# Shizheng-Wen/GAOT-3D

Hardware: AMD Instinct MI355X
Metric: mesh-points/sec fwd+bwd, 500K-pt DrivAerNet++ sample (higher is better)
Workload: dtype bf16; 1 GPU; configs[1]: one 500000-point car-like surface sample, latent 64x64x32, knn k=8 encoder + flipped decoder, C=32 P=2 d=256 h=8 F=1024 L=10 rope, attention dropout 0.1 (training mode), MSE + AdamW step; CSR build and geoembed stats inside the step (a decoder list that is the encoder's with its rows swapped shares the encoder's two lists); points=500000, edges=4000000, edges_decoder=4000000, layers=10, precision=bf16, points_per_gpu=500000, point_order=random

## Files before the change

gaot_3d_amd/_lib.py:

```python
from __future__ import annotations

import ctypes as C
import os

_HERE = os.path.dirname(os.path.abspath(__file__))
LIB_PATH = os.environ.get("GAOT_LIB") or os.path.join(_HERE, "lib", "libgaot3d_hip.so")

MAX_MLP_LAYERS = 5


class GaotError(RuntimeError):
    pass


class MlpT(C.Structure):
    _fields_ = [("n_hidden", C.c_int), ("hidden", C.c_int), ("channels", C.c_int),
                ("weight", C.c_void_p * MAX_MLP_LAYERS), ("bias", C.c_void_p * MAX_MLP_LAYERS)]


class MlpGradT(C.Structure):
    _fields_ = [("weight", C.c_void_p * MAX_MLP_LAYERS), ("bias", C.c_void_p * MAX_MLP_LAYERS)]


_lib = None

_p, _i, _i64, _sz, _f, _d = C.c_void_p, C.c_int, C.c_int64, C.c_size_t, C.c_float, C.c_double

SIGNATURES = {
    "gaot_abi_version": (_i, []),
    "gaot_last_error": (C.c_char_p, []),
    "gaot_launch_count": (_i64, [_i]),
    "gaot_csr_workspace_bytes": (_sz, [_i64, _i64]),
    "gaot_csr_build": (_i, [_p, _i, _i64, _i, _i64, _p, _p, _p, _p, _p, _sz, _p]),
    "gaot_gno_fwd_workspace_bytes": (_sz, [_i64, _i]),
    "gaot_gno_fwd": (_i, [C.POINTER(MlpT), _p, _p, _p, _p, _p, _p, _i64, _i64, _p, _i, _p, _sz, _p]),
    "gaot_gno_bwd_workspace_bytes": (_sz, [C.POINTER(MlpT), _i64, _i64]),
    "gaot_gno_bwd": (_i, [C.POINTER(MlpT), _p, _p, _p, _p, _p, _p, _p, _p, _i64, _i64, _i64, _p,
                          C.POINTER(MlpGradT), _i, _p, _sz, _p]),
    "gaot_gno_bwd_coords": (_i, [C.POINTER(MlpT), _p, _p, _p, _p, _p, _p, _p, _p, _i64, _i64, _i64, _p,
                                 C.POINTER(MlpGradT), _p, _i, _p, _sz, _p]),
    "gaot_geoembed_stats_workspace_bytes": (_sz, []),
    "gaot_geoembed_moments": (_i, [_p, _p, _p, _p, _i64, _p, _p]),
    "gaot_geoembed_from_moments": (_i, [_p, _i64, _p, _p, _sz, _p]),
    "gaot_geoembed_raw": (_i, [_p, _p, _p, _p, _i64, _p, _p, _p, _sz, _p]),
    "gaot_geoembed_finalize": (_i, [_p, _i64, _p, _i64, _p, _sz, _p]),
    "gaot_geoembed_from_moments_bwd_workspace_bytes": (_sz, [_i64]),
    "gaot_geoembed_from_moments_bwd": (_i, [_p, _p, _i64, _p, _p, _sz, _p]),
    "gaot_geoembed_moments_bwd": (_i, [_p, _p, _p, _p, _i64, _p, _p, _p, _p]),
    "gaot_gemm_workspace_bytes": (_sz, [_i64, _i64, _i64]),
    "gaot_gemm": (_i, [_p, _p, _p, _i64, _i64, _i64, _i64, _i64, _i64, _i, _i, _p, _i, _p, _i64, _p, _i, _p, _sz, _p]),
    "gaot_gemm_ex": (_i, [_p, _p, _p, _i64, _i64, _i64, _i64, _i64, _i64, _i, _i, _i, _i, _i, _p, _i, _p, _i64, _p, _i, _p,
                          _sz, _p]),
    "gaot_attn_fwd": (_i, [_p, _p, _p, _p, _p, _i64, _i64, _i64, _i64, _i, _i, _i, _i, _i, _f, _f, _p, _i, _i, _i, _p]),
    "gaot_attn_bwd": (_i, [_p] * 10 + [_i64] * 8 + [_i, _i, _i, _i, _i, _f, _f, _p, _i, _i, _i, _i, _p]),
    "gaot_attn_bwd_fused_f32_scratch_bytes": (_i64, [_i, _i, _i]),
    "gaot_attn_bwd_fused_f32": (_i, [_p] * 10 + [_i64] * 8 + [_i, _i, _i, _i, _i, _f, _f, _p, _i, _i, _i, _p, C.c_size_t, _p]),
    "gaot_attn_dropout_mask": (_i, [_p, _f, _i, _i, _i, _p, _p]),
    "gaot_dropout_seed_next": (_i, [_p, C.c_uint64, _p, _p]),
    "gaot_dropout_seed_block": (_i, [_p, C.c_uint64, _i, _p, _p]),
    "gaot_attn_bf16_image_bytes": (_sz, [_i, _i, _i, _i]),
    "gaot_rope_table": (_i, [_p, _i, _i, _p, _p]),
    "gaot_qkv_image": (_i, [_p, _p, _p, _i64, _i64, _i64, _i, _i, _i, _p, _f, _p]),
    "gaot_qkv_image_packed": (_i, [_p, _p, _p, _i64, _i64, _i64, _i64, _i, _i, _p, _f, _i, _p]),
    "gaot_pack_heads": (_i, [_p, _p, _i64, _i, _i, _i, _p, _p, _i, _i, _i, _p]),
    "gaot_attn_bwd_bf16_scratch_bytes": (_sz, [_i, _i, _i, _i]),
    "gaot_attn_bwd_bf16_fused_eligible": (_i, [_i, _i, _i, _i]),
    "gaot_attn_fwd_bf16": (_i, [_p, _p, _p, _p, _p, _i, _i, _i, _i, _i, _f, _f, _p, _i, _i, _p]),
    "gaot_attn_bwd_bf16": (_i, [_p, _p, _p, _p, _p, _p, _p, _p, _i, _i, _i, _i, _i, _f, _f, _p, _i, _i, _i, _p]),
    "gaot_rmsnorm_fwd": (_i, [_p, _p, _p, _p, _p, _i64, _i, _f, _p]),
    "gaot_rmsnorm_bwd_workspace_bytes": (_sz, [_i64, _i]),
    "gaot_rmsnorm_bwd": (_i, [_p, _p, _p, _p, _p, _p, _p, _i64, _i, _p, _sz, _p]),
    "gaot_rmsnorm_bwd2": (_i, [_p, _p, _p, _p, _p, _p, _p, _p, _i64, _i, _p, _sz, _p]),
    "gaot_colsum_workspace_bytes": (_sz, [_i64, _i64]),
    "gaot_colsum": (_i, [_p, _i64, _i64, _i64, _p, _p, _sz, _p]),
    "gaot_gemm_ex_partials": (_i, [_p, _p, _p, _i64, _i64, _i64, _i64, _i64, _i64, _i, _i, _i, _i, _i, _p, _sz, _p, _p, _p]),
    "gaot_rmsnorm_bwd_parts": (_i64, [_i64]),
    "gaot_colsum_parts": (_i64, [_i64]),
    "gaot_reduce_multi": (_i, [_p, _i, _p]),
    "gaot_rope": (_i, [_p, _i64, _i64, _i, _i, _i, _i, _p, _i, _p]),
    "gaot_swiglu_fwd": (_i, [_p, _p, _i64, _i, _p]),
    "gaot_swiglu_bwd": (_i, [_p, _p, _p, _i64, _i, _p]),
    "gaot_adamw_step": (_i, [_p, _i, _p, _p, _d, _d, _d, _d, _p]),
    "gaot_mlp2_fwd": (_i, [_p, _i64, _i, _i, _i, _p, _p, _p, _p, _p, _p]),
    "gaot_mlp2_bwd_workspace_bytes": (_sz, [_i, _i]),
    "gaot_mlp2_bwd": (_i, [_p, _i64, _i, _i, _i, _p, _p, _p, _p, _p, _p, _p, _p, _p, _sz, _p]),
    "gaot_knn_grid": (_i, [_p, _i64, _p, _p, _i, _p, _p]),
    "gaot_radius_grid_count": (_i, [_p, _i64, _p, _p, _f, _i, _p, _p]),
    "gaot_radius_grid_fill": (_i, [_p, _i64, _p, _p, _f, _i, _p, _p, _p, _p]),
    "gaot_knn_brute": (_i, [_p, _i64, _p, _i64, _i, _p, _p]),
    "gaot_radius_brute_count": (_i, [_p, _i64, _p, _i64, _f, _i, _p, _p]),
    "gaot_radius_brute_fill": (_i, [_p, _i64, _p, _i64, _f, _i, _p, _p, _p, _p]),
    "gaot_exclusive_scan_workspace_bytes": (_sz, [_i64]),
    "gaot_exclusive_scan_i32": (_i, [_p, _i64, _p, _p, _sz, _p]),
    "gaot_segment_cap_flags": (_i, [_p, _p, _i64, _i, _p, _p]),
    "gaot_unique_pair_flags": (_i, [_p, _p, _i64, _p, _p]),
    "gaot_random_keep_flags": (_i, [_p, _i64, _d, _p, _p]),
    "gaot_dropout": (_i, [_p, _p, _d, _i64, _p, _p]),
    "gaot_segment_random_cap_flags": (_i, [_p, _p, _p, _i64, _i, _p, _p]),
    "gaot_compact_pairs": (_i, [_p, _p, _p, _p, _i64, _p, _p, _p]),
    "gaot_cast_bf16": (_i, [_p, _p, _i64, _p]),
    "gaot_cast_bf16_multi": (_i, [_p, _i, _p]),
    "gaot_cast_bf16_transpose_multi": (_i, [_p, _p, _p, _i, _p]),
    "gaot_swiglu_fwd_bf16": (_i, [_p, _p, _i64, _i, _p]),
    "gaot_ffn_w13_swiglu": (_i, [_p, _p, _p, _p, _i64, _i64, _i64, _i, _p]),
    "gaot_ffn_w2_bwd_swiglu": (_i, [_p, _p, _p, _p, _i64, _i64, _i64, _i, _p]),
    "gaot_swiglu_bwd_bf16": (_i, [_p, _p, _p, _i64, _i, _p]),
    "gaot_ffn_packed_bytes": (_i64, [_i, _i]),
    "gaot_ffn_pack": (_i, [_p, _p, _i, _p, _i, _p]),
    "gaot_ffn_pack_multi": (_i, [_p, _i, _i, _i, _p]),
    "gaot_ffn_fwd": (_i, [_p, _p, _p, _i64, _p, _p, _p, _i64, _i, _p]),
    "gaot_norm_ffn_fwd": (_i, [_p, _i64, _p, _f, _p, _p, _p, _p, _i64, _i, _p]),
    "gaot_block_packed_bytes": (_i64, [_i]),
    "gaot_block_pack_multi": (_i, [_p, _i, _i, _p]),
    "gaot_block_tail_fwd": (_i, [_p, _i64, _p, _i64, _p, _f, _p, _p, _p, _p, _p, _i64, _i, _p]),
    "gaot_qkv_packed_bytes": (_i64, [_i64, _i]),
    "gaot_qkv_pack_multi": (_i, [_p, _i, _i64, _i, _p]),
    "gaot_norm_qkv_image": (_i, [_p, _i64, _p, _f, _p, _p, _p, _p, _i64, _i, _i, _i, _p, _f, _p]),
    "gaot_skip_packed_bytes": (_i64, []),
    "gaot_skip_pack_multi": (_i, [_p, _i, _p]),
    "gaot_cat_norm_qkv_image": (_i, [_p, _i64, _p, _i64, _p, _p, _p, _p, _f, _p, _p, _p, _p, _i64, _i, _i, _i, _p, _f, _p]),
    "gaot_norm_bwd_parts": (_i64, [_i64]),
    "gaot_ffn_bwd_norm": (_i, [_p, _p, _p, _p, _i64, _p, _p, _p, _p, _p, _p, _p, _i64, _i, _p]),
    "gaot_qkv_bwd_norm": (_i, [_p, _i64, _p, _p, _i64, _p, _p, _p, _p, _p, _p, _i64, _p]),
    "gaot_qkv_bwd_norm_cat": (_i, [_p, _i64, _p, _p, _i64, _p, _p, _p, _p, _p, _p, _p, _i, _p, _i64, _p]),
    "gaot_oproj_bwd_image": (_i, [_p, _p, _p, _i, _p, _p, _i64, _i, _p]),
    "gaot_ffn_bwd_dag": (_i, [_p, _p, _p, _p, _p, _p, _i64, _i, _p]),
    "gaot_ffn_bwd": (_i, [_p, _p, _p, _p, _p, _p, _p, _i, _i64, _i, _p]),
    "gaot_act_bwd": (_i, [_p, _p, _p, _i64, _i, _p]),
    "gaot_act_fwd": (_i, [_p, _p, _i64, _i, _p]),
    "gaot_axpy": (_i, [_p, _p, _f, _p, _i64, _i64, _p]),
    "gaot_stream_copy": (_i, [_p, _p, _i64, _p]),
    "gaot_stream_copy_ex": (_i, [_p, _p, _i64, _i, _p]),
    "gaot_patchify": (_i, [_p, _p, _i, _i, _i, _i, _i, _i, _i, _p]),
    "gaot_mse_workspace_bytes": (_sz, []),
    "gaot_mse_fwd": (_i, [_p, _p, _i64, _p, _p, _sz, _p]),
    "gaot_mse_bwd": (_i, [_p, _p, _i64, _p, _p, _p]),
    "gaot_gather_rows": (_i, [_p, _i64, _p, _i64, _i, _p, _i64, _p]),
    "gaot_segment_reduce": (_i, [_p, _i64, _p, _p, _i64, _i, _i, _p, _p, _p]),
    "gaot_segment_reduce_bwd": (_i, [_p, _p, _p, _p, _i64, _i64, _i, _i, _p, _p]),
    "gaot_segment_softmax_fwd": (_i, [_p, _p, _i64, _p, _p]),
    "gaot_segment_softmax_bwd": (_i, [_p, _p, _p, _i64, _p, _p]),
    "gaot_edge_coords": (_i, [_p, _p, _p, _p, _i64, _i, _p, _i64, _p]),
    "gaot_mul": (_i, [_p, _p, _i64, _i, _i, _p, _p]),
    "gaot_mul_rowsum": (_i, [_p, _p, _i64, _i, _p, _p]),
    "gaot_affine_cols": (_i, [_p, _p, _p, _i64, _i, _p, _p]),
    "gaot_scale_mix_fwd": (_i, [_p, _i, _p, _p, _p, _i64, _i, _p]),
    "gaot_scale_mix_bwd": (_i, [_p, _i, _p, _p, _p, _p, _i64, _i, _p]),
}


def load():
    global _lib
    if _lib is not None:
        return _lib
    if not os.path.exists(LIB_PATH):
        raise GaotError(f"{LIB_PATH} not found: build it with `python -c 'import __graft_entry__ as g; g.build()'` "
                        f"or `make -C gaot_3d_amd/csrc` (there is no CPU/PyTorch fallback)")
    lib = C.CDLL(LIB_PATH)
    for name, (res, args) in SIGNATURES.items():
        fn = getattr(lib, name)
        fn.restype = res
        fn.argtypes = args
    if lib.gaot_abi_version() != 11:
        raise GaotError("libgaot3d_hip.so ABI version mismatch")
    _lib = lib
    return lib


def check(rc: int, what: str):
    if rc != 0:
        msg = load().gaot_last_error()
        raise GaotError(f"{what} failed (code {rc}): {msg.decode() if msg else ''}")
```

gaot_3d_amd/functional.py:

```python
from __future__ import annotations

import os
from typing import List, Optional

import torch
from torch.autograd import Function

from . import ops
from ._lib import GaotError

Tensor = torch.Tensor


def _w2d(w: Tensor) -> Tensor:
    if w.dim() == 3:
        w = w[:, :, 0]
    return w if w.is_contiguous() else w.contiguous()


_WB_CACHE: dict = {}


def _wb_eligible(w: Tensor, prec: int) -> bool:
    n, k = w.shape
# ... 763 lines not shown
            packed = ops.qkv_pack_multi([wcat32], True)[0]
        spk = _SKIP_PACK_CACHE.get((wsk.data_ptr(), tuple(wsk.shape)))
        if spk is None:
            spk = ops.skip_pack_multi([wsk])[0]
        freqs, b, s, h, hkv, scale = image_spec
        img, xo, yb, rstd = ops.cat_norm_qkv_image(xa, xb, spk, bskip, norm_w, eps, packed, b, s, h, hkv, freqs, scale)
        out = torch.empty(1, dtype=torch.float32, device=x.device).expand(m, ntot)
        out._gaot_qkv_image = img
        ctx.save_for_backward(xa, xb, xo, norm_w, rstd, yb, _wb(wcat32, 1), packed, _wb(wsk, 1), spk)
        ctx.wparams, ctx.nparam, ctx.sparams = tuple(weights), norm_w, (wskip, bskip)
        ctx.meta = (x.shape, skip.shape, [w.shape for w in weights], ntot, wskip.shape)
        ctx.set_materialize_grads(False)
        return out, xo.view(x.shape)

    @staticmethod
    def backward(ctx, dqkv: Tensor, dres: Optional[Tensor] = None):
        xa, xb, xo, norm_w, rstd, yb, wcat, packed, wskb, spk = ctx.saved_tensors
        xshape, sshape, wshapes, ntot, wsshape = ctx.meta
        m = xa.shape[0]
        d = dqkv if dqkv.is_contiguous() else dqkv.contiguous()
        dwcat = _dw_gemm(d, yb, ntot, 256, m, ntot, 256, 1, ctx.wparams)
        dres2 = None if dres is None else dres.reshape(m, 256)
        dxa = dxb = None
        fused_dx = _NORM_BWD_FUSED and _CAT_BWD_DX and ctx.needs_input_grad[0] and (ctx.same or ctx.needs_input_grad[1])
        if fused_dx:
            dxo, dxa, dxb, dnw = ops.qkv_bwd_norm_cat(d, packed, xo, norm_w, rstd, dres2, spk, ctx.same, defer=ops.defer_ok((ctx.nparam,)))
        elif _NORM_BWD_FUSED:
            dxo, dnw = ops.qkv_bwd_norm(d, packed, xo, norm_w, rstd, dres2, None, defer=ops.defer_ok((ctx.nparam,)))
        else:
            dn = ops.gemm(d, wcat, m, 256, ntot, ntot, 256, False, False, precision=1)
            dxo, dnw = ops.rmsnorm_bwd(xo, norm_w, dn, rstd, dres2, defer=ops.defer_ok((ctx.nparam,)))
        n, k = 256, 512
        wsk, bsk = ctx.sparams
        if not fused_dx:
            dxa = ops.gemm(dxo, wskb, m, 256, n, n, k, False, False, precision=1) if (ctx.needs_input_grad[0] or ctx.same) else None
            if ctx.same and ctx.needs_input_grad[0]:
                dxa = ops.gemm(dxo, wskb[:, 256:], m, 256, n, n, k, False, False, residual=dxa, ldr=256, precision=1)
            else:
                dxb = ops.gemm(dxo, wskb[:, 256:], m, 256, n, n, k, False, False, precision=1) if ctx.needs_input_grad[1] else None
        dws = torch.empty(n, k, dtype=torch.float32, device=d.device)
        ops.gemm(dxo, xa, n, 256, m, n, 256, True, False, out=dws, ldc=k, precision=1)
        ops.gemm(dxo, xb, n, 256, m, n, 256, True, False, out=dws[:, 256:], ldc=k, precision=1)
        dbs = ops.colsum(dxo, m, n, n) if (bsk is not None and ctx.needs_input_grad[3]) else None
        dwl, col = [], 0
        for shp in wshapes:
            dwl.append(dwcat[col:col + shp[0]].view(shp))
            col += shp[0]
        return (None if dxa is None else dxa.view(xshape), None if dxb is None else dxb.view(sshape), dws.view(wsshape), dbs, dnw, None, None, *dwl)


class BlockTailFn(Function):

    @staticmethod
    def enabled() -> bool:
        return _FFN_FUSED and _NORM_FFN and _BLOCK_TAIL and ops.get_precision() == "bf16"

    @staticmethod
    def eligible(x: Tensor, wo: Tensor, norm_w: Tensor, w1: Tensor, w3: Tensor, w2: Tensor) -> bool:
        wo2 = _w2d(wo)
        return (BlockTailFn.enabled() and tuple(wo2.shape) == (256, 256) and wo2.dtype == torch.float32 and wo.requires_grad
                and NormFFNFn.eligible(x, norm_w, w1, w3, w2))

    @staticmethod
    def forward(ctx, o: Tensor, x: Tensor, wo: Tensor, norm_w: Tensor, eps: float, w1: Tensor, w3: Tensor, w2: Tensor, attn_dims=None):
        ctx.attn_dims = attn_dims if (attn_dims is not None and _OPROJ_BWD_IMAGE and attn_dims[2] == 8 and attn_dims[0] * attn_dims[1] == o.shape[0]) else None
        f, d = w1.shape
        o2 = o if o.is_contiguous() else o.contiguous()
        x2 = x if x.is_contiguous() else x.contiguous()
        wo2 = _w2d(wo)
        wcat32 = w1.new_empty(0).set_(w1.untyped_storage(), w1.storage_offset(), (2 * f, d), (d, 1))
        key = (wcat32.data_ptr(), tuple(wcat32.shape))
        packed, _has_bwd = _FFN_PACK_CACHE.get(key, (None, False))
        if packed is None or _WO_PACKED.get(key) != wo2.data_ptr():
            packed = ops.block_pack_multi([(wcat32, _w2d(w2), wo2)], f)[0]
        y, h, yb, rstd = ops.block_tail_fwd(o2, x2, norm_w, eps, packed, f)
        ctx.save_for_backward(o2, _wb(wo2, 1), h, norm_w, rstd, yb, packed)
        ctx.wparams = (w1, w3, w2)
        ctx.nparam, ctx.oparam = norm_w, wo
        ctx.meta = (f, d, w1.shape, w2.shape, wo.shape)
        return y

    @staticmethod
    def backward(ctx, dy: Tensor):
        o2, wob, h, norm_w, rstd, yb, packed = ctx.saved_tensors
        f, d, w1shape, w2shape, woshape = ctx.meta
        m = h.shape[0]
        dy2 = dy if dy.is_contiguous() else dy.contiguous()
        if _NORM_BWD_FUSED:
            dh, dag, u, dyb, dnw = ops.ffn_bwd_norm(yb, dy2, packed, f, h, norm_w, rstd, defer=ops.defer_ok((ctx.nparam,)))
        else:
            dn, dag, u, dyb = ops.ffn_bwd(yb, dy2, packed, f, True)
            dh, dnw = ops.rmsnorm_bwd(h, norm_w, dn, rstd, defer=ops.defer_ok((ctx.nparam,)))
        dw2 = _dw_gemm(dyb, u, d, f, m, d, f, 1, ctx.wparams[2:]).view(w2shape)
        dwcat = _dw_gemm(dag, yb, 2 * f, d, m, 2 * f, d, 1, ctx.wparams[:2])
        d_o = None
        if ctx.needs_input_grad[0]:
            if ctx.attn_dims is not None:
                b_, s_, h_, hkv_ = ctx.attn_dims
                img, delta = ops.oproj_bwd_image(dh, o2, packed, f, b_, s_, h_, hkv_)
                d_o = torch.empty(1, dtype=torch.float32, device=dh.device).expand(m, d)
                d_o._gaot_do_image = (img, delta)
            else:
                d_o = ops.gemm(dh, wob, m, d, d, d, d, False, False, precision=1)
        dwo = _dw_gemm(dh, o2, d, d, m, d, d, 1, (ctx.oparam,)).view(woshape)
        return d_o, (dh if ctx.needs_input_grad[1] else None), dwo, dnw, None, dwcat[:f].view(w1shape), dwcat[f:].view(w1shape), dw2, None


class Mlp2Fn(Function):

    @staticmethod
    def eligible(x: Tensor, fcs, non_linearity: str) -> bool:
        if len(fcs) != 2 or non_linearity != "gelu" or ops.get_precision() != "bf16" or not x.is_cuda:
            return False
        w1, w2 = _w2d(fcs[0].weight), _w2d(fcs[1].weight)
        return (x.shape[-1] == 32 and w1.shape[1] == 32 and w1.shape[0] in (64, 128, 256) and 1 <= w2.shape[0] <= 4
                and w2.shape[1] == w1.shape[0] and fcs[0].bias is not None and x.dtype == torch.float32)

    @staticmethod
    def forward(ctx, x: Tensor, w1: Tensor, b1: Tensor, w2: Tensor, b2: Optional[Tensor]):
        x2 = x.reshape(-1, x.shape[-1])
        if not x2.is_contiguous():
            x2 = x2.contiguous()
        w1c, w2c = _w2d(w1), _w2d(w2)
        out = ops.mlp2_forward(x2, w1c, b1, w2c, b2)
        ctx.save_for_backward(x2, w1c, b1, w2c)
        ctx.meta = (x.shape, w1.shape, w2.shape, b2 is not None)
        return out.view(*x.shape[:-1], w2c.shape[0])

    @staticmethod
    def backward(ctx, dout: Tensor):
        x2, w1c, b1, w2c = ctx.saved_tensors
        xshape, w1shape, w2shape, has_b2 = ctx.meta
        d = dout.reshape(x2.shape[0], w2c.shape[0])
        if not d.is_contiguous():
            d = d.contiguous()
        dx, dw1, db1, dw2 = ops.mlp2_backward(x2, w1c, b1, w2c, d)
        db2 = ops.colsum(d, d.shape[0], d.shape[1], d.shape[1]) if has_b2 else None
        return dx.view(xshape), dw1.view(w1shape), db1, dw2.view(w2shape), db2


class AddFn(Function):

    @staticmethod
    def forward(ctx, a: Tensor, b: Tensor, period: Optional[int]):
        ac = a if a.is_contiguous() else a.contiguous()
        bc = b if b.is_contiguous() else b.contiguous()
        ctx.period = period
        return ops.axpy(ac, bc, 1.0, period)

    @staticmethod
    def backward(ctx, g: Tensor):
        if ctx.period is not None and ctx.needs_input_grad[1]:
            raise GaotError("AddFn: gradient of a broadcast addend is not needed on the hot path")
        return g, (g if ctx.period is None else None), None


def add(a: Tensor, b: Tensor) -> Tensor:
    return AddFn.apply(a, b, None)


class PatchifyFn(Function):
    @staticmethod
    def forward(ctx, x: Tensor, b, d, h, w, p, c, to_tokens: bool):
        ctx.args = (b, d, h, w, p, c, to_tokens)
        xc = x if x.is_contiguous() else x.contiguous()
        return ops.patchify(xc, b, d, h, w, p, c, to_tokens)

    @staticmethod
    def backward(ctx, g: Tensor):
        b, d, h, w, p, c, to_tokens = ctx.args
        gc = g if g.is_contiguous() else g.contiguous()
        return ops.patchify(gc, b, d, h, w, p, c, not to_tokens), None, None, None, None, None, None, None


class MSELossFn(Function):
    @staticmethod
    def forward(ctx, pred: Tensor, target: Tensor):
        p = pred if pred.is_contiguous() else pred.contiguous()
        t = target if target.is_contiguous() else target.contiguous()
        if p.shape != t.shape:
            raise GaotError(f"mse_loss: shape mismatch {tuple(p.shape)} vs {tuple(t.shape)}")
        ctx.save_for_backward(p, t)
        return ops.mse_fwd(p, t)

    @staticmethod
    def backward(ctx, g: Tensor):
        p, t = ctx.saved_tensors
        gl = g if g.is_contiguous() else g.contiguous()
        return ops.mse_bwd(p, t, gl), None


def mse_loss(pred: Tensor, target: Tensor) -> Tensor:
    return MSELossFn.apply(pred, target)


def _adjacent(ws) -> bool:
    k = ws[0].shape[1]
    for a, b in zip(ws[:-1], ws[1:]):
        if b.shape[1] != k or not (a.is_contiguous() and b.is_contiguous()) or a.device != b.device:
            return False
        if b.data_ptr() != a.data_ptr() + a.numel() * a.element_size():
            return False
        if a.untyped_storage().data_ptr() != b.untyped_storage().data_ptr():
            return False
    return True


def colocate(params) -> None:
    ps = list(params)
    if _adjacent([_w2d(p.data) for p in ps]):
        return
    if torch.cuda.is_available() and torch.cuda.is_current_stream_capturing():
        raise GaotError("colocate: parameters must be co-located before the step is captured into a graph")
    with torch.no_grad():
        flat = torch.empty(sum(p.numel() for p in ps), dtype=ps[0].dtype, device=ps[0].device)
        off = 0
        for p in ps:
            v = flat[off:off + p.numel()].view(p.shape)
            v.copy_(p.data)
            p.data = v
            off += p.numel()


class MultiLinearFn(Function):

    @staticmethod
    def forward(ctx, x: Tensor, precision: Optional[int], image_spec, *weights: Tensor):
        ws = [_w2d(w) for w in weights]
        k = ws[0].shape[1]
        x2 = x.reshape(-1, k)
        if not x2.is_contiguous():
            x2 = x2.contiguous()
        m = x2.shape[0]
        ntot = sum(w.shape[0] for w in ws)
        ctx.fused = len(ws) > 1 and _adjacent(ws) and all(ctx.needs_input_grad[3 + i] for i in range(len(ws)))
        ctx.wparams = tuple(weights)
        if ctx.fused:
            wcat = _wb(ws[0].new_empty(0).set_(ws[0].untyped_storage(), ws[0].storage_offset(), (ntot, k), (k, 1)), precision)
            xb = bf16_copy_of(x, (m, k)) if wcat.dtype == torch.bfloat16 else None
            xa = xb if xb is not None else x2
            if image_spec is not None and xb is not None and k == 256 and ntot % 64 == 0:
                freqs, b, s, h, hkv, scale = image_spec
                img = ops.qkv_image(xb, wcat, m, b, s, h, hkv, freqs, scale)
                out = torch.empty(1, dtype=torch.float32, device=x.device).expand(m, ntot)
                out._gaot_qkv_image = img
                ctx.save_for_backward(xa, wcat)
                ctx.precision, ctx.xshape, ctx.wshapes = precision, x.shape, [w.shape for w in weights]
                return out
            out = torch.empty(m, ntot, dtype=torch.float32, device=x.device)
            ops.gemm(xa, wcat, m, ntot, k, k, k, False, True, out=out, ldc=ntot, precision=precision)
            ctx.save_for_backward(xa, wcat)
        else:
            out = torch.empty(m, ntot, dtype=torch.float32, device=x.device)
            col = 0
            for w in ws:
                n = w.shape[0]
                ops.gemm(x2, w, m, n, k, k, k, False, True, out=out[:, col:], ldc=ntot, precision=precision)
                col += n
            ctx.save_for_backward(x2, *ws)
        ctx.precision, ctx.xshape, ctx.wshapes = precision, x.shape, [w.shape for w in weights]
        return out

    @staticmethod
    def backward(ctx, dout: Tensor):
        x2, *ws = ctx.saved_tensors
        m, k = x2.shape
        d = dout if dout.is_contiguous() else dout.contiguous()
        ntot = d.shape[1]
        dx = None
        dws = []
        col = 0
        if ctx.fused:
            (wcat,) = ws
            if ctx.needs_input_grad[0]:
                dx = ops.gemm(d, wcat, m, k, ntot, ntot, k, False, False, precision=ctx.precision)
            dwcat = _dw_gemm(d, x2, ntot, k, m, ntot, k, ctx.precision, ctx.wparams)
            for shp in ctx.wshapes:
                n = shp[0]
                dws.append(dwcat[col:col + n].view(shp))
                col += n
            return (dx.view(ctx.xshape) if dx is not None else None, None, None, *dws)
        for i, w in enumerate(ws):
            n = w.shape[0]
            blk = d[:, col:]
            if ctx.needs_input_grad[0]:
                dx = ops.gemm(blk, w, m, k, n, ntot, k, False, False, residual=dx, ldr=k, precision=ctx.precision)
            dws.append(_dw_gemm(blk, x2, n, k, m, ntot, k, ctx.precision, ctx.wparams[i:i + 1]).view(ctx.wshapes[i])
                       if ctx.needs_input_grad[3 + i] else None)
            col += n
        return (dx.view(ctx.xshape) if dx is not None else None, None, None, *dws)


def multi_linear(x: Tensor, weights, precision: Optional[int] = None, image_spec=None) -> Tensor:
    return MultiLinearFn.apply(x, precision, image_spec, *weights)


def _same_view(a: Tensor, b: Tensor) -> bool:
    if a is b:
        return True
    ba, bb = (a._base if a._base is not None else a), (b._base if b._base is not None else b)
    return ba is bb and a.data_ptr() == b.data_ptr() and a.shape == b.shape and a.stride() == b.stride()


class CatLinearFn(Function):

    @staticmethod
    def forward(ctx, weight: Tensor, bias: Optional[Tensor], precision: Optional[int], *xs: Tensor):
        w = _w2d(weight)
        n, k = w.shape
        xs2 = [x if x.is_contiguous() else x.contiguous() for x in xs]
        if sum(x.shape[1] for x in xs2) != k:
            raise GaotError(f"cat_linear: inputs have {sum(x.shape[1] for x in xs2)} features, weight expects {k}")
        m = xs2[0].shape[0]
        if all(x.shape[1] > 64 and x.shape[1] % 8 == 0 for x in xs2):
            w = _wb(w, precision)
        y = None
        col = 0
        for i, x in enumerate(xs2):
            ki = x.shape[1]
            y = ops.gemm(x, w[:, col:], m, n, ki, ki, k, False, True, bias if i == 0 else None, 0, residual=y, ldr=n,
                         precision=precision)
            col += ki
        ctx.save_for_backward(w, *xs2)
        ctx.meta = (precision, weight.shape, bias is not None)
        ctx.dups = any(_same_view(xs[i], xs[j]) for i in range(len(xs)) for j in range(i))
        return y

    @staticmethod
    def backward(ctx, dy: Tensor):
        w, *xs = ctx.saved_tensors
        precision, wshape, has_bias = ctx.meta
        n, k = w.shape
        d = dy if dy.is_contiguous() else dy.contiguous()
        m = d.shape[0]
        dw = torch.empty(n, k, dtype=torch.float32, device=d.device) if ctx.needs_input_grad[0] else None
        dxs = []
        col = 0
        first = {}
        for i, x in enumerate(xs):
            ki = x.shape[1]
            key = (x.data_ptr(), tuple(x.shape))
            j = first.get(key)
            if ctx.needs_input_grad[3 + i] and j is not None and dxs[j] is not None and ctx.dups:
                dxs[j] = ops.gemm(d, w[:, col:], m, ki, n, n, k, False, False, residual=dxs[j], ldr=ki, precision=precision)
                dxs.append(None)
            else:
                dxs.append(ops.gemm(d, w[:, col:], m, ki, n, n, k, False, False, precision=precision)
                           if ctx.needs_input_grad[3 + i] else None)
                first.setdefault(key, i)
            if dw is not None:
                ops.gemm(d, x, n, ki, m, n, ki, True, False, out=dw[:, col:], ldc=k, precision=precision)
            col += ki
        db = ops.colsum(d, m, n, n) if (has_bias and ctx.needs_input_grad[1]) else None
        return (dw.view(wshape) if dw is not None else None, db, None, *dxs)


def cat_linear(xs, weight, bias=None, precision: Optional[int] = None) -> Tensor:
    return CatLinearFn.apply(weight, bias, precision, *xs)


class ScaleMixFn(Function):

    @staticmethod
    def forward(ctx, logits: Tensor, *xs: Tensor):
        xc = [x if x.is_contiguous() else x.contiguous() for x in xs]
        lg = logits if logits.is_contiguous() else logits.contiguous()
        out, w = ops.scale_mix_fwd(xc, lg)
        ctx.save_for_backward(w, *xc)
        return out

    @staticmethod
    def backward(ctx, dout: Tensor):
        w, *xs = ctx.saved_tensors
        d = dout if dout.is_contiguous() else dout.contiguous()
        dxs, dlog = ops.scale_mix_bwd(xs, w, d)
        return (dlog, *dxs)
```

gaot_3d_amd/model/layers/geoembed.py:

```python
from typing import Optional

import torch
import torch.nn as nn

from ... import edgeops as EO
from ... import functional as GF
from ... import ops
from .integral_transform import coords_need_grad, graph_for


class GeoStatFn(torch.autograd.Function):

    @staticmethod
    def forward(ctx, source_pos, query_pos, g):
        mom = ops.geoembed_moments(source_pos, query_pos, g)
        ctx.g = g
        ctx.save_for_backward(source_pos, query_pos, mom)
        return ops.geoembed_from_moments(mom)

    @staticmethod
    def backward(ctx, d):
        source_pos, query_pos, mom = ctx.saved_tensors
        g = ctx.g
        adj = ops.geoembed_from_moments_bwd(mom, d)
        ge, gq = ops.geoembed_moments_bwd(source_pos, query_pos, g, adj)
        gs = None
        if ctx.needs_input_grad[0]:
            gs, _ = EO.coord_grads_by_endpoint(ge, g, 0, None, source_pos.shape[0], query_pos.shape[0])
        return gs, (gq if ctx.needs_input_grad[1] else None), None


class GeometricEmbedding(nn.Module):
    def __init__(self, input_dim, output_dim, method="statistical", pooling="max", **kwargs):
        super().__init__()
        self.input_dim = input_dim
        self.output_dim = output_dim
        self.method = method.lower()
        self.pooling = pooling.lower()
        self.kwargs = kwargs
        if self.pooling not in ["max", "mean"]:
            raise ValueError(f"Unsupported pooling method: {self.pooling}. Supported methods: 'max', 'mean'.")
        if self.method == "statistical":
            self.mlp = nn.Sequential(nn.Linear(3 + 2 * input_dim, 64), nn.ReLU(), nn.Linear(64, output_dim))
        elif self.method == "pointnet":
            self.pointnet_mlp = nn.Sequential(nn.Linear(input_dim, 32), nn.ReLU(), nn.Linear(32, 32), nn.ReLU())
            self.fc = nn.Sequential(nn.Linear(32, output_dim))
        else:
            raise ValueError(f"Unknown method: {self.method}")

    def forward(self, source_pos, query_pos, edge_index, batch_source: Optional[torch.Tensor] = None,
                batch_query: Optional[torch.Tensor] = None, neighbors_counts: Optional[torch.Tensor] = None,
                graph=None, shard_group=None, sharded_queries_total: Optional[int] = None):
        if graph is None:
            graph = graph_for(edge_index.to(query_pos.device), source_pos.shape[0], query_pos.shape[0])
        coord_grad = coords_need_grad(source_pos, query_pos)
        if shard_group is not None and coord_grad:
            raise NotImplementedError("GeometricEmbedding: gradients with respect to the coordinates are not supported for "
                                      "point-sharded samples (shard_group); detach the coordinates")
        if self.method == "pointnet":
            if shard_group is not None and sharded_queries_total is None:
                return self._forward_pointnet_sharded(source_pos, query_pos, graph, shard_group)
            return self._forward_pointnet(source_pos, query_pos, graph)
        if shard_group is not None and sharded_queries_total is not None:
            feats = ops.geoembed_stats_sharded_queries(source_pos, query_pos, graph, shard_group, sharded_queries_total)
        elif shard_group is not None:
            import torch.distributed as dist
            mom = ops.geoembed_moments(source_pos, query_pos, graph)
            from ... import comm
            comm.run(lambda: dist.all_reduce(mom, op=dist.ReduceOp.SUM, group=shard_group), (mom,), "all_reduce")
            feats = ops.geoembed_from_moments(mom)
        elif coord_grad:
            feats = GeoStatFn.apply(source_pos, query_pos, graph)
        else:
            ent = graph.__dict__.get("_geo_feats")
            if (ent is not None and ent[0] is source_pos and ent[1] == source_pos._version and ent[2] is query_pos
                    and ent[3] == query_pos._version):
                feats = ent[4]
            else:
                feats = ops.geoembed_from_moments(ops.geoembed_moments(source_pos, query_pos, graph))
                graph.__dict__["_geo_feats"] = (source_pos, source_pos._version, query_pos, query_pos._version, feats)
        h = GF.linear(feats, self.mlp[0].weight, self.mlp[0].bias, act="relu", precision=0)
        return GF.linear(h, self.mlp[2].weight, self.mlp[2].bias, precision=0)

    def _forward_pointnet_sharded(self, source_pos, query_pos, g, group):
        from ...sharding import GlobalSegmentMaxFn, GlobalSegmentMeanFn
        nq = query_pos.shape[0]
        rp = g.by_dst.rowptr
        deg = (rp[1:] - rp[:-1]).to(torch.float32)
        if g.by_dst.num_edges == 0:
            local = torch.zeros(nq, 32, dtype=query_pos.dtype, device=query_pos.device)
        else:
            c = EO.edge_coords(source_pos, query_pos, g, 1)
            h = GF.linear(c, self.pointnet_mlp[0].weight, self.pointnet_mlp[0].bias, act="relu", precision=0)
            h = GF.linear(h, self.pointnet_mlp[2].weight, self.pointnet_mlp[2].bias, act="relu", precision=0)
            local = EO.SegmentReduceFn.apply(h, g, EO.MAX if self.pooling == "max" else EO.MEAN)
        if self.pooling == "max":
            pooled, gdeg = GlobalSegmentMaxFn.apply(local, deg, group)
        else:
            pooled = GlobalSegmentMeanFn.apply(local, deg, group)
            gdeg = deg.clone()
            import torch.distributed as dist
            from ... import comm
            comm.run(lambda: dist.all_reduce(gdeg, op=dist.ReduceOp.SUM, group=group), (gdeg,), "all_reduce")
        po = GF.linear(pooled, self.fc[0].weight, self.fc[0].bias, precision=0)
        return EO.RowScaleFn.apply(po, (gdeg > 0).to(torch.float32))

    def _forward_pointnet(self, source_pos, query_pos, g):
        nq = query_pos.shape[0]
        if g.by_dst.num_edges == 0:
            return torch.zeros(nq, self.output_dim, dtype=query_pos.dtype, device=query_pos.device)
        c = EO.EdgeOffsetFn.apply(source_pos, query_pos, g)
        h = GF.linear(c, self.pointnet_mlp[0].weight, self.pointnet_mlp[0].bias, act="relu", precision=0)
        h = GF.linear(h, self.pointnet_mlp[2].weight, self.pointnet_mlp[2].bias, act="relu", precision=0)
        pooled = EO.SegmentReduceFn.apply(h, g, EO.MAX if self.pooling == "max" else EO.MEAN)
        po = GF.linear(pooled, self.fc[0].weight, self.fc[0].bias, precision=0)
        rp = g.by_dst.rowptr
        has = (rp[1:] > rp[:-1]).to(torch.float32)
        return EO.RowScaleFn.apply(po, has)
```

gaot_3d_amd/model/layers/magno.py:

```python
from dataclasses import dataclass, field
from typing import Any, List, Optional, Tuple, Union

import torch
import torch.nn as nn

from ... import functional as GF
from ...data import coalesce_edges, knn_edges_bruteforce, radius_edges_bruteforce
from .geoembed import GeometricEmbedding
from ...graph import apply_neighbor_sampling
from .integral_transform import IntegralTransform, graph_for
from .mlp import ChannelMLP, LinearChannelMLP


@dataclass
class MAGNOConfig:
    use_gno: bool = True
    gno_coord_dim: int = 2
    gno_radius: float = 0.033
    lifting_channels: int = 16
    encoder_feature_attr: Any = "x"
    in_gno_channel_mlp_hidden_layers: list = field(default_factory=lambda: [64, 64, 64])
    in_gno_transform_type: str = "linear"
    projection_channels: int = 256
    out_gno_channel_mlp_hidden_layers: list = field(default_factory=lambda: [64, 64])
    out_gno_transform_type: str = "linear"
    mlp_type: str = "channel"
    scales: list = field(default_factory=lambda: [1.0])
    use_scale_weights: bool = False
    use_graph_cache: bool = True
    gno_use_torch_cluster: bool = False
    gno_use_torch_scatter: str = True
    node_embedding: bool = False
    use_attn: Optional[bool] = None
    attention_type: str = "cosine"
    use_geoembed: Any = field(default_factory=lambda: [True, True])
    embedding_method: str = "statistical"
    pooling: str = "max"
    sampling_strategy: Optional[str] = None
    max_neighbors: Optional[int] = None
    sample_ratio: Optional[float] = None
    neighbor_strategy: Any = "radius"
    k_neighbors: int = 1
    precompute_edges: bool = True
    asynchronous_graph_building: bool = False


def parse_neighbor_strategy(neighbor_strategy: Union[str, List[str]]) -> Tuple[str, str]:
    if isinstance(neighbor_strategy, str):
        return neighbor_strategy, neighbor_strategy
    if isinstance(neighbor_strategy, (list, tuple)) and len(neighbor_strategy) == 2:
        return neighbor_strategy[0], neighbor_strategy[1]
    raise ValueError(f"neighbor_strategy must be str or list of length 2, got {neighbor_strategy}")


def parse_geoembed_strategy(use_geoembed: Union[bool, List[bool]]) -> Tuple[bool, bool]:
    if isinstance(use_geoembed, bool):
        return use_geoembed, use_geoembed
    if isinstance(use_geoembed, (list, tuple)) and len(use_geoembed) == 2:
        return use_geoembed[0], use_geoembed[1]
    raise ValueError(f"use_geoembed must be bool or list of length 2, got {use_geoembed}")


def _per_graph(fn, phys_pos, batch_idx_phys, latent_pos, batch_idx_latent):
    nb = int(batch_idx_phys.max().item()) + 1 if batch_idx_phys.numel() else 1
    out = []
    for b in range(nb):
        pm = (batch_idx_phys == b).nonzero(as_tuple=True)[0]
        lm = (batch_idx_latent == b).nonzero(as_tuple=True)[0]
        e = fn(phys_pos[pm], latent_pos[lm])
        out.append((e, pm, lm))
    return out


def get_neighbor_strategy(neighbor_strategy: str, phys_pos, batch_idx_phys, latent_tokens_pos, batch_idx_latent,
                          radius: float, k_neighbors: int = 1, is_decoder: bool = False, latent_dims=None):
    if phys_pos.is_cuda:
        from ... import graph as device_graph
        return device_graph.get_neighbor_strategy(neighbor_strategy, phys_pos, batch_idx_phys, latent_tokens_pos,
                                                  batch_idx_latent, radius, k_neighbors, is_decoder, latent_dims=latent_dims)

    def enc(strategy, p, l):
        knn = rad = None
        if strategy in ("knn", "bidirectional"):
            knn = knn_edges_bruteforce(p, l, k_neighbors)
        if strategy in ("radius", "bidirectional"):
            rad = radius_edges_bruteforce(p, l, radius, 32, centers="latent")
        if strategy == "knn":
            return knn
        if strategy == "radius":
            return rad
        if strategy == "bidirectional":
            return coalesce_edges(torch.cat([knn, rad], dim=1), l.shape[0])
        raise ValueError(f"Unknown encoder strategy: {strategy}")

    def dec(strategy, p, l):
        if strategy == "reverse":
            return enc("bidirectional", p, l).flip(0)
        knn = rad = None
        if strategy in ("knn", "bidirectional"):
            knn = knn_edges_bruteforce(p, l, k_neighbors).flip(0)
        if strategy in ("radius", "bidirectional"):
            rad = radius_edges_bruteforce(p, l, radius, 32, centers="phys")
        if strategy == "knn":
            return knn
        if strategy == "radius":
            return rad
        if strategy == "bidirectional":
            return coalesce_edges(torch.cat([knn, rad], dim=1), p.shape[0])
        raise ValueError(f"Unknown decoder strategy: {strategy}")

    parts = _per_graph((lambda p, l: dec(neighbor_strategy, p, l)) if is_decoder else
                       (lambda p, l: enc(neighbor_strategy, p, l)),
                       phys_pos, batch_idx_phys, latent_tokens_pos, batch_idx_latent)
    outs = []
    for e, pm, lm in parts:
        if is_decoder:
            outs.append(torch.stack([lm[e[0]], pm[e[1]]]))
        else:
            outs.append(torch.stack([pm[e[0]], lm[e[1]]]))
    return torch.cat(outs, dim=1) if outs else torch.empty((2, 0), dtype=torch.long, device=phys_pos.device)


def _make_mlp(mlp_type, layers):
    if mlp_type == "linear":
        return LinearChannelMLP(layers=layers)
    if len(layers) == 2:
        return ChannelMLP(in_channels=layers[0], out_channels=layers[1], n_layers=1)
    return ChannelMLP(in_channels=layers[0], out_channels=layers[-1], hidden_channels=layers[1], n_layers=len(layers) - 1,
                      n_dim=1)


def _check_unsupported(cfg: MAGNOConfig):
    if cfg.sampling_strategy not in (None, "max_neighbors", "ratio"):
        raise ValueError(f"Invalid sampling strategy: {cfg.sampling_strategy}")


def _sample(module, edge_index, num_query):
    if module.sampling_strategy is None:
        return edge_index
    from ...graph import apply_neighbor_sampling
    return apply_neighbor_sampling(edge_index, num_query, edge_index.device, module.sampling_strategy, module.max_neighbors,
                                   module.sample_ratio, module.training)


def _sum_scales(outs):
    acc = outs[0]
    for o in outs[1:]:
        acc = GF.add(acc, o)
    return acc


def _make_scale_weighting(coord_dim, num_scales):
    return nn.Sequential(nn.Linear(coord_dim, 16), nn.ReLU(), nn.Linear(16, num_scales))


def _mix_scales(module, outs, pos):
    if len(outs) == 1:
        return outs[0]
    if not module.use_scale_weights:
        return _sum_scales(outs)
    sw = module.scale_weighting
    h = GF.linear(pos, sw[0].weight, sw[0].bias, act="relu", precision=0)
    logits = GF.linear(h, sw[2].weight, sw[2].bias, precision=0)
    return GF.ScaleMixFn.apply(logits, *outs)


class MAGNOEncoder(nn.Module):
    def __init__(self, in_channels, out_channels, gno_config: MAGNOConfig):
        super().__init__()
        _check_unsupported(gno_config)
        self.sampling_strategy = gno_config.sampling_strategy
        self.max_neighbors = gno_config.max_neighbors
        self.sample_ratio = gno_config.sample_ratio
        self.gno_radius = gno_config.gno_radius
        self.scales = gno_config.scales
        self.lifting_channels = gno_config.lifting_channels
        self.coord_dim = gno_config.gno_coord_dim
        self.feature_attr_name = gno_config.encoder_feature_attr
        self.precompute_edges = gno_config.precompute_edges
        self.mlp_type = gno_config.mlp_type
        self.encoder_strategy, self.decoder_strategy = parse_neighbor_strategy(gno_config.neighbor_strategy)
        self.k_neighbors = gno_config.k_neighbors
        self.use_gno = gno_config.use_gno
        if self.use_gno:
            kin = self.coord_dim * 2
            if gno_config.in_gno_transform_type in ("nonlinear", "nonlinear_kernelonly"):
                kin += in_channels
            layers = [kin] + list(gno_config.in_gno_channel_mlp_hidden_layers) + [self.lifting_channels]
            self.gno = IntegralTransform(channel_mlp_layers=layers, transform_type=gno_config.in_gno_transform_type,
                                         use_attn=gno_config.use_attn, coord_dim=self.coord_dim,
                                         attention_type=gno_config.attention_type)
            self.lifting = _make_mlp(gno_config.mlp_type, [in_channels, self.lifting_channels])
        else:
            self.gno = None
            self.lifting = None
        self.use_geoembed = parse_geoembed_strategy(gno_config.use_geoembed)[0]
        if self.use_geoembed:
            self.geoembed = GeometricEmbedding(input_dim=self.coord_dim, output_dim=self.lifting_channels,
                                               method=gno_config.embedding_method, pooling=gno_config.pooling)
            self.recovery = _make_mlp(gno_config.mlp_type, [2 * self.lifting_channels, self.lifting_channels])
        self.use_scale_weights = gno_config.use_scale_weights
        if self.use_scale_weights:
            self.num_scales = len(self.scales)
            self.scale_weighting = _make_scale_weighting(self.coord_dim, self.num_scales)
            self.scale_weight_activation = nn.Softmax(dim=-1)

    def _features(self, batch):
        names = self.feature_attr_name if isinstance(self.feature_attr_name, (list, tuple)) else [self.feature_attr_name]
        feats = []
        for a in names:
            f = getattr(batch, a, None)
            if f is None:
                if self.use_gno:
                    raise AttributeError(f"MAGNOEncoder requires feature attribute '{a}' but it was not found in the batch.")
            else:
                feats.append(f)
        return feats

    def forward(self, batch, latent_tokens_pos: torch.Tensor, latent_tokens_batch_idx: torch.Tensor) -> torch.Tensor:
        phys_pos = batch.pos
        device = phys_pos.device
        num_graphs = batch.num_graphs
        m_per_graph = latent_tokens_pos.shape[0] // num_graphs
        phys_feat = self._features(batch)
        lifted = None
        if self.use_gno:
            if len(self.lifting.fcs) == 1 and not (self.training and getattr(self.lifting, "dropout_p", 0.0) > 0.0):
                lifted = GF.cat_linear(phys_feat, self.lifting.fcs[0].weight, self.lifting.fcs[0].bias, precision=0)
            else:
                lifted = self.lifting.forward_rows(phys_feat[0] if len(phys_feat) == 1 else torch.cat(phys_feat, dim=1))
        outs = []
        for si, scale in enumerate(self.scales):
            if self.precompute_edges:
                attr = f"encoder_edge_index_s{si}"
                if not hasattr(batch, attr):
                    raise AttributeError(f"Batch object missing pre-computed '{attr}'")
                edge_index = getattr(batch, attr).to(device)
            else:
                edge_index = get_neighbor_strategy(self.encoder_strategy, phys_pos, batch.batch, latent_tokens_pos,
                                                   latent_tokens_batch_idx, self.gno_radius * scale, self.k_neighbors,
                                                   False, latent_dims=getattr(self, "latent_dims", None)).to(device)
            edge_index = _sample(self, edge_index, latent_tokens_pos.shape[0])
            g = graph_for(edge_index, phys_pos.shape[0], latent_tokens_pos.shape[0],
                          batch if self.sampling_strategy is None else None, ("enc", si))
            enc = self.gno(y_pos=phys_pos, x_pos=latent_tokens_pos, edge_index=edge_index, f_y=lifted,
                           graph=g) if self.use_gno else None
            shard_group = getattr(self, "_shard_group", None)
            if shard_group is not None and enc is not None:
                from ...sharding import GlobalSegmentMeanFn
                deg = (g.by_dst.rowptr[1:] - g.by_dst.rowptr[:-1]).to(enc.dtype)
                enc = GlobalSegmentMeanFn.apply(enc, deg, shard_group)
            geo = self.geoembed(phys_pos, latent_tokens_pos, edge_index, graph=g, shard_group=shard_group) \
                if self.use_geoembed else None
            if enc is not None and geo is not None:
                enc = GF.cat_linear([enc, geo], self.recovery.fcs[0].weight, self.recovery.fcs[0].bias, precision=0)
            elif enc is None and geo is not None:
                enc = geo
            elif enc is None:
                raise ValueError("GNO and GeoEmbed are both disabled. No encoding will be performed.")
            outs.append(enc)
        out = _mix_scales(self, outs, latent_tokens_pos)
        return out.view(num_graphs, m_per_graph, self.lifting_channels)


class MAGNODecoder(nn.Module):
    def __init__(self, in_channels, out_channels, gno_config: MAGNOConfig):
        super().__init__()
        _check_unsupported(gno_config)
        self.sampling_strategy = gno_config.sampling_strategy
        self.max_neighbors = gno_config.max_neighbors
        self.sample_ratio = gno_config.sample_ratio
        self.gno_radius = gno_config.gno_radius
        self.scales = gno_config.scales
        self.coord_dim = gno_config.gno_coord_dim
        self.in_channels = in_channels
        self.out_channels = out_channels
        self.use_geoembed = parse_geoembed_strategy(gno_config.use_geoembed)[1]
        self.use_scale_weights = gno_config.use_scale_weights
        self.precompute_edges = gno_config.precompute_edges
        self.mlp_type = gno_config.mlp_type
        self.encoder_strategy, self.decoder_strategy = parse_neighbor_strategy(gno_config.neighbor_strategy)
        self.k_neighbors = gno_config.k_neighbors
        kin = self.coord_dim * 2
        if gno_config.out_gno_transform_type in ("nonlinear", "nonlinear_kernelonly"):
            kin += in_channels
        layers = [kin] + list(gno_config.out_gno_channel_mlp_hidden_layers) + [in_channels]
        self.gno = IntegralTransform(channel_mlp_layers=layers, transform_type=gno_config.out_gno_transform_type,
                                     use_attn=gno_config.use_attn, coord_dim=self.coord_dim,
                                     attention_type=gno_config.attention_type)
        self.projection = _make_mlp(gno_config.mlp_type, [in_channels, gno_config.projection_channels, out_channels])
        if self.use_geoembed:
            self.geoembed = GeometricEmbedding(input_dim=self.coord_dim, output_dim=in_channels,
                                               method=gno_config.embedding_method, pooling=gno_config.pooling)
            self.recovery = _make_mlp(gno_config.mlp_type, [2 * in_channels, in_channels])
        if self.use_scale_weights:
            self.num_scales = len(self.scales)
            self.scale_weighting = _make_scale_weighting(self.coord_dim, self.num_scales)
            self.scale_weight_activation = nn.Softmax(dim=-1)

    def forward(self, rndata_flat, phys_pos_query, batch_idx_phys_query, latent_tokens_pos, latent_tokens_batch_idx,
                batch=None) -> torch.Tensor:
        device = rndata_flat.device
        outs = []
        for si, scale in enumerate(self.scales):
            if self.precompute_edges:
                attr = f"decoder_edge_index_s{si}"
                if not hasattr(batch, attr):
                    raise AttributeError(f"Batch object missing pre-computed '{attr}'")
                edge_index = getattr(batch, attr).to(device)
            else:
                edge_index = get_neighbor_strategy(self.decoder_strategy, phys_pos_query, batch_idx_phys_query,
                                                   latent_tokens_pos, latent_tokens_batch_idx, self.gno_radius * scale,
                                                   self.k_neighbors, True,
                                                   latent_dims=getattr(self, "latent_dims", None)).to(device)
            edge_index = _sample(self, edge_index, phys_pos_query.shape[0])
            g = graph_for(edge_index, latent_tokens_pos.shape[0], phys_pos_query.shape[0],
                          batch if self.sampling_strategy is None else None, ("dec", si))
            dec = self.gno(y_pos=latent_tokens_pos, x_pos=phys_pos_query, edge_index=edge_index, f_y=rndata_flat, graph=g)
            if self.use_geoembed:
                sg = getattr(self, "_shard_group", None)
                if sg is not None:
                    total = getattr(batch, "shard", (0, 0, 0, 0, phys_pos_query.shape[0]))[4]
                    geo = self.geoembed(latent_tokens_pos, phys_pos_query, edge_index, graph=g, shard_group=sg,
                                        sharded_queries_total=total)
                else:
                    geo = self.geoembed(latent_tokens_pos, phys_pos_query, edge_index, graph=g)
                dec = GF.cat_linear([dec, geo], self.recovery.fcs[0].weight, self.recovery.fcs[0].bias, precision=0)
            outs.append(dec)
        return self.projection.forward_rows(_mix_scales(self, outs, phys_pos_query))
```

gaot_3d_amd/ops.py:

```python
from __future__ import annotations

import ctypes as C
import functools
import os
from dataclasses import dataclass
from typing import List, Optional, Sequence, Tuple

import torch

from . import _lib
from ._lib import GaotError, MlpGradT, MlpT, check

Tensor = torch.Tensor


_raw_stream = getattr(torch._C, "_cuda_getCurrentRawStream", None)


def _stream() -> C.c_void_p:
    if _raw_stream is not None:
        return C.c_void_p(_raw_stream(torch.cuda.current_device()))
    return C.c_void_p(torch.cuda.current_stream().cuda_stream)


# ... 893 lines not shown
        raise GaotError("norm_qkv_image: fp32 [b * s, 256] input expected")
    nw = _req(norm_weight, torch.float32, "norm_weight")
    img = _ws(lib.gaot_attn_bf16_image_bytes(b, s, h, hkv), x.device)
    yb = torch.empty(rows, 256, dtype=torch.bfloat16, device=x.device)
    rstd = torch.empty(rows, dtype=torch.float32, device=x.device)
    table = rope_table(freqs, s) if freqs is not None else None
    with _timed("norm_qkv_image"):
        check(lib.gaot_norm_qkv_image(_ptr(x), x.stride(0), _ptr(nw), float(eps), _ptr(packed), _ptr(img), _ptr(yb), _ptr(rstd), rows, s, h, hkv,
                                      _ptr(table), _qscale(scale), _stream()), "gaot_norm_qkv_image")
    return img, yb, rstd


def _finish_parts(part: Tensor, n: int, parts: int, lanes: int, defer: bool) -> Tensor:
    out = torch.empty(n, dtype=torch.float32, device=part.device)
    if defer:
        _defer(part, out, n, parts, lanes)
        return out
    arr = (_ReduceDesc * 1)()
    arr[0].part, arr[0].out, arr[0].n, arr[0].parts, arr[0].lanes = part.data_ptr(), out.data_ptr(), n, parts, lanes
    check(_lib.load().gaot_reduce_multi(arr, 1, _stream()), "gaot_reduce_multi")
    return out


def ffn_bwd_norm(yb: Tensor, dy: Tensor, packed: Tensor, f: int, h: Tensor, norm_weight: Tensor, rstd: Tensor, defer: bool = False):
    lib = _lib.load()
    rows = yb.shape[0]
    if yb.dtype != torch.bfloat16 or not yb.is_contiguous() or yb.shape[1] != 256:
        raise GaotError("ffn_bwd_norm: contiguous bf16 [rows, 256] input expected")
    if dy.dtype != torch.float32 or not dy.is_contiguous() or tuple(dy.shape) != (rows, 256):
        raise GaotError("ffn_bwd_norm: contiguous fp32 [rows, 256] gradient expected")
    if h.dtype != torch.float32 or tuple(h.shape) != (rows, 256) or h.stride(1) != 1:
        raise GaotError("ffn_bwd_norm: fp32 [rows, 256] norm input expected")
    nw = _req(norm_weight, torch.float32, "norm_weight")
    dev = yb.device
    dag = torch.empty(rows, 2 * f, dtype=torch.bfloat16, device=dev)
    u = torch.empty(rows, f, dtype=torch.bfloat16, device=dev)
    dyb = torch.empty(rows, 256, dtype=torch.bfloat16, device=dev)
    dh = torch.empty(rows, 256, dtype=torch.float32, device=dev)
    parts = int(lib.gaot_norm_bwd_parts(rows))
    part = torch.empty(parts, 256, dtype=torch.float32, device=dev)
    with _timed("ffn_bwd_norm"):
        check(lib.gaot_ffn_bwd_norm(_ptr(yb), _ptr(dy), _ptr(packed), _ptr(h), h.stride(0), _ptr(nw), _ptr(rstd), _ptr(dag), _ptr(u), _ptr(dyb),
                                    _ptr(dh), _ptr(part), rows, int(f), _stream()), "gaot_ffn_bwd_norm")
    return dh, dag, u, dyb, _finish_parts(part, 256, parts, 32, defer)


def qkv_bwd_norm(dqkv: Tensor, packed: Tensor, x: Tensor, norm_weight: Tensor, rstd: Tensor, dres: Optional[Tensor] = None,
                 dtap: Optional[Tensor] = None, defer: bool = False):
    lib = _lib.load()
    rows, n = dqkv.shape
    if dqkv.dtype != torch.float32 or not dqkv.is_contiguous() or n % 256:
        raise GaotError("qkv_bwd_norm: contiguous fp32 [rows, N] gradient with N a multiple of 256 expected")
    if x.dtype != torch.float32 or tuple(x.shape) != (rows, 256) or x.stride(1) != 1:
        raise GaotError("qkv_bwd_norm: fp32 [rows, 256] norm input expected")
    nw = _req(norm_weight, torch.float32, "norm_weight")
    dres = None if dres is None else _req(dres, torch.float32, "dres")
    dtap = None if dtap is None else _req(dtap, torch.float32, "dtap")
    dev = dqkv.device
    dx = torch.empty(rows, 256, dtype=torch.float32, device=dev)
    parts = int(lib.gaot_norm_bwd_parts(rows))
    part = torch.empty(parts, 256, dtype=torch.float32, device=dev)
    with _timed("qkv_bwd_norm"):
        check(lib.gaot_qkv_bwd_norm(_ptr(dqkv), n, _ptr(packed), _ptr(x), x.stride(0), _ptr(nw), _ptr(rstd), _ptr(dres), _ptr(dtap), _ptr(dx),
                                    _ptr(part), rows, _stream()), "gaot_qkv_bwd_norm")
    return dx, _finish_parts(part, 256, parts, 32, defer)


def qkv_bwd_norm_cat(dqkv: Tensor, packed: Tensor, x: Tensor, norm_weight: Tensor, rstd: Tensor, dres: Optional[Tensor], skip_packed: Tensor,
                     same: bool, defer: bool = False):
    lib = _lib.load()
    rows, n = dqkv.shape
    if dqkv.dtype != torch.float32 or not dqkv.is_contiguous() or n % 256:
        raise GaotError("qkv_bwd_norm_cat: contiguous fp32 [rows, N] gradient with N a multiple of 256 expected")
    if x.dtype != torch.float32 or tuple(x.shape) != (rows, 256) or x.stride(1) != 1:
        raise GaotError("qkv_bwd_norm_cat: fp32 [rows, 256] norm input expected")
    if skip_packed.numel() != int(lib.gaot_skip_packed_bytes()):
        raise GaotError("qkv_bwd_norm_cat: skip_packed is not a skip_pack_multi image")
    nw = _req(norm_weight, torch.float32, "norm_weight")
    dres = None if dres is None else _req(dres, torch.float32, "dres")
    dev = dqkv.device
    dx = torch.empty(rows, 256, dtype=torch.float32, device=dev)
    dxa = torch.empty(rows, 256, dtype=torch.float32, device=dev)
    dxb = None if same else torch.empty(rows, 256, dtype=torch.float32, device=dev)
    parts = int(lib.gaot_norm_bwd_parts(rows))
    part = torch.empty(parts, 256, dtype=torch.float32, device=dev)
    with _timed("qkv_bwd_norm_cat"):
        check(lib.gaot_qkv_bwd_norm_cat(_ptr(dqkv), n, _ptr(packed), _ptr(x), x.stride(0), _ptr(nw), _ptr(rstd), _ptr(dres), _ptr(skip_packed),
                                        _ptr(dx), _ptr(dxa), _ptr(dxb), int(bool(same)), _ptr(part), rows, _stream()), "gaot_qkv_bwd_norm_cat")
    return dx, dxa, dxb, _finish_parts(part, 256, parts, 32, defer)


def oproj_bwd_image(dh: Tensor, attn_out: Tensor, packed: Tensor, f: int, b: int, s: int, h: int, hkv: int):
    lib = _lib.load()
    rows = dh.shape[0]
    if h != 8 or rows != b * s or any(t.dtype != torch.float32 or not t.is_contiguous() or tuple(t.shape) != (rows, 256) for t in (dh, attn_out)):
        raise GaotError("oproj_bwd_image: contiguous fp32 [b * s, 256] tensors and 8 heads of 32 expected")
    scratch = attn_bwd_scratch(b, s, h, hkv, dh.device)
    delta = torch.empty(b, h, s, dtype=torch.float32, device=dh.device)
    with _timed("oproj_bwd_image"):
        check(lib.gaot_oproj_bwd_image(_ptr(dh), _ptr(attn_out), _ptr(packed), int(f), _ptr(scratch), _ptr(delta), rows, int(s), _stream()),
              "gaot_oproj_bwd_image")
    return scratch, delta


def norm_ffn_fwd(h: Tensor, norm_weight: Tensor, eps: float, packed: Tensor, f: int):
    lib = _lib.load()
    if h.dtype != torch.float32 or h.dim() != 2 or h.shape[1] != 256 or h.stride(1) != 1:
        raise GaotError("norm_ffn_fwd: fp32 [rows, 256] input expected")
    nw = _req(norm_weight, torch.float32, "norm_weight")
    rows = h.shape[0]
    y = torch.empty(rows, 256, dtype=torch.float32, device=h.device)
    yb = torch.empty(rows, 256, dtype=torch.bfloat16, device=h.device)
    rstd = torch.empty(rows, dtype=torch.float32, device=h.device)
    with _timed("norm_ffn_fwd"):
        check(lib.gaot_norm_ffn_fwd(_ptr(h), h.stride(0), _ptr(nw), float(eps), _ptr(packed), _ptr(y), _ptr(yb), _ptr(rstd), rows, int(f),
                                    _stream()), "gaot_norm_ffn_fwd")
    return y, yb, rstd


def ffn_bwd_dag(xb: Tensor, dy: Tensor, packed: Tensor, f: int, want_dyb: bool = True):
    lib = _lib.load()
    if xb.dtype != torch.bfloat16 or not xb.is_contiguous() or xb.shape[1] != 256:
        raise GaotError("ffn_bwd_dag: contiguous bf16 [rows, 256] input expected")
    rows = xb.shape[0]
    if dy.dtype != torch.float32 or not dy.is_contiguous() or tuple(dy.shape) != (rows, 256):
        raise GaotError("ffn_bwd_dag: contiguous fp32 [rows, 256] gradient expected")
    dag = torch.empty(rows, 2 * f, dtype=torch.bfloat16, device=xb.device)
    u = torch.empty(rows, f, dtype=torch.bfloat16, device=xb.device)
    dyb = torch.empty(rows, 256, dtype=torch.bfloat16, device=xb.device) if want_dyb else None
    with _timed("ffn_bwd_dag"):
        check(lib.gaot_ffn_bwd_dag(_ptr(xb), _ptr(dy), _ptr(packed), _ptr(dag), _ptr(u), _ptr(dyb), rows, int(f), _stream()), "gaot_ffn_bwd_dag")
    return dag, u, dyb


def ffn_bwd(xb: Tensor, dy: Tensor, packed: Tensor, f: int, add_dy: bool, want_dyb: bool = True):
    lib = _lib.load()
    if xb.dtype != torch.bfloat16 or not xb.is_contiguous() or xb.shape[1] != 256:
        raise GaotError("ffn_bwd: contiguous bf16 [rows, 256] input expected")
    rows = xb.shape[0]
    if dy.dtype != torch.float32 or not dy.is_contiguous() or tuple(dy.shape) != (rows, 256):
        raise GaotError("ffn_bwd: contiguous fp32 [rows, 256] gradient expected")
    dag = torch.empty(rows, 2 * f, dtype=torch.bfloat16, device=xb.device)
    u = torch.empty(rows, f, dtype=torch.bfloat16, device=xb.device)
    dyb = torch.empty(rows, 256, dtype=torch.bfloat16, device=xb.device) if want_dyb else None
    dx = torch.empty(rows, 256, dtype=torch.float32, device=xb.device)
    with _timed("ffn_bwd"):
        check(lib.gaot_ffn_bwd(_ptr(xb), _ptr(dy), _ptr(packed), _ptr(dag), _ptr(u), _ptr(dyb), _ptr(dx), int(add_dy), rows, int(f), _stream()),
              "gaot_ffn_bwd")
    return dx, dag, u, dyb


def ffn_w2_bwd_swiglu(dyb: Tensor, w2t: Tensor, ag: Tensor, f: int) -> Tensor:
    lib = _lib.load()
    if any(t.dtype != torch.bfloat16 or not t.is_contiguous() for t in (dyb, w2t, ag)):
        raise GaotError("ffn_w2_bwd_swiglu: contiguous bf16 operands expected")
    dag = torch.empty_like(ag)
    with _timed("ffn_w2_bwd_swiglu"):
        check(lib.gaot_ffn_w2_bwd_swiglu(_ptr(dyb), _ptr(w2t), _ptr(ag), _ptr(dag), dyb.shape[0], dyb.shape[1], w2t.shape[1], int(f),
                                         _stream()), "gaot_ffn_w2_bwd_swiglu")
    return dag


def swiglu_bwd_bf16(ag: Tensor, du: Tensor, f: int) -> Tensor:
    lib = _lib.load()
    dag = torch.empty_like(ag)
    check(lib.gaot_swiglu_bwd_bf16(_ptr(ag), _ptr(du), _ptr(dag), ag.shape[0], f, _stream()), "gaot_swiglu_bwd_bf16")
    return dag


def patchify(src: Tensor, b: int, d: int, h: int, w: int, p: int, c: int, to_tokens: bool) -> Tensor:
    lib = _lib.load()
    dst = torch.empty_like(src)
    check(lib.gaot_patchify(_ptr(src), _ptr(dst), b, d, h, w, p, c, int(to_tokens), _stream()), "gaot_patchify")
    return dst


def mse_fwd(pred: Tensor, target: Tensor) -> Tensor:
    lib = _lib.load()
    loss = torch.empty((), dtype=torch.float32, device=pred.device)
    ws = _ws(lib.gaot_mse_workspace_bytes(), pred.device)
    check(lib.gaot_mse_fwd(_ptr(pred), _ptr(target), pred.numel(), _ptr(loss), _ptr(ws), ws.numel(), _stream()),
          "gaot_mse_fwd")
    return loss


def mse_bwd(pred: Tensor, target: Tensor, grad_loss: Tensor) -> Tensor:
    lib = _lib.load()
    dp = torch.empty_like(pred)
    check(lib.gaot_mse_bwd(_ptr(pred), _ptr(target), pred.numel(), _ptr(grad_loss), _ptr(dp), _stream()), "gaot_mse_bwd")
    return dp


def geoembed_stats_sharded_queries(source_pos: Tensor, query_pos: Tensor, g: BipartiteGraph, group, num_queries_total: int) -> Tensor:
    import torch.distributed as dist
    lib = _lib.load()
    source_pos = _req(source_pos, torch.float32, "source_pos")
    query_pos = _req(query_pos, torch.float32, "query_pos")
    if source_pos.shape[1] != 3:
        raise GaotError("geoembed statistical features: coord_dim must be 3 on the HIP path")
    q = g.num_dst
    feat = torch.empty(q, 9, dtype=torch.float32, device=query_pos.device)
    sums = torch.empty(18, dtype=torch.float64, device=query_pos.device)
    ws = _ws(lib.gaot_geoembed_stats_workspace_bytes(), query_pos.device)
    check(lib.gaot_geoembed_raw(_ptr(source_pos), _ptr(query_pos), _ptr(g.by_dst.rowptr), _ptr(g.by_dst.other), q, _ptr(feat),
                                _ptr(sums), _ptr(ws), ws.numel(), _stream()), "gaot_geoembed_raw")
    if group is not None:
        from . import comm
        comm.run(lambda: dist.all_reduce(sums, op=dist.ReduceOp.SUM, group=group), (sums,), "all_reduce")
    check(lib.gaot_geoembed_finalize(_ptr(feat), q, _ptr(sums), int(num_queries_total), _ptr(ws), ws.numel(), _stream()),
          "gaot_geoembed_finalize")
    return feat


def geoembed_moments(source_pos: Tensor, query_pos: Tensor, g: BipartiteGraph) -> Tensor:
    lib = _lib.load()
    source_pos = _req(source_pos, torch.float32, "source_pos")
    query_pos = _req(query_pos, torch.float32, "query_pos")
    if source_pos.shape[1] != 3:
        raise GaotError("geoembed statistical features: coord_dim must be 3 on the HIP path")
    mom = torch.empty(g.num_dst, 12, dtype=torch.float64, device=query_pos.device)
    check(lib.gaot_geoembed_moments(_ptr(source_pos), _ptr(query_pos), _ptr(g.by_dst.rowptr), _ptr(g.by_dst.other), g.num_dst,
                                    _ptr(mom), _stream()), "gaot_geoembed_moments")
    return mom


def geoembed_from_moments(mom: Tensor) -> Tensor:
    lib = _lib.load()
    q = mom.shape[0]
    feat = torch.empty(q, 9, dtype=torch.float32, device=mom.device)
    ws = _ws(lib.gaot_geoembed_stats_workspace_bytes(), mom.device)
    check(lib.gaot_geoembed_from_moments(_ptr(mom), q, _ptr(feat), _ptr(ws), ws.numel(), _stream()), "gaot_geoembed_from_moments")
    return feat


def geoembed_from_moments_bwd(mom: Tensor, grad_feat: Tensor) -> Tensor:
    lib = _lib.load()
    q = mom.shape[0]
    grad_feat = _req(grad_feat, torch.float32, "grad_features")
    adj = torch.empty(q, 12, dtype=torch.float64, device=mom.device)
    ws = _ws(lib.gaot_geoembed_from_moments_bwd_workspace_bytes(q), mom.device)
    check(lib.gaot_geoembed_from_moments_bwd(_ptr(mom), _ptr(grad_feat), q, _ptr(adj), _ptr(ws), ws.numel(), _stream()),
          "gaot_geoembed_from_moments_bwd")
    return adj


def geoembed_moments_bwd(source_pos: Tensor, query_pos: Tensor, g: BipartiteGraph, adj: Tensor):
    lib = _lib.load()
    source_pos = _req(source_pos, torch.float32, "source_pos")
    query_pos = _req(query_pos, torch.float32, "query_pos")
    ge = torch.empty(g.by_dst.num_edges, 3, dtype=torch.float32, device=query_pos.device)
    gq = torch.empty(g.num_dst, 3, dtype=torch.float32, device=query_pos.device)
    check(lib.gaot_geoembed_moments_bwd(_ptr(source_pos), _ptr(query_pos), _ptr(g.by_dst.rowptr), _ptr(g.by_dst.other),
                                        g.num_dst, _ptr(adj), _ptr(ge), _ptr(gq), _stream()), "gaot_geoembed_moments_bwd")
    return ge, gq


def _ptr_array(ts):
    arr = (C.c_void_p * len(ts))()
    for i, t in enumerate(ts):
        arr[i] = _ptr(t).value
    return arr


def scale_mix_fwd(xs, logits: Tensor):
    lib = _lib.load()
    n, c = xs[0].shape
    out = torch.empty_like(xs[0])
    w = torch.empty(n, len(xs), dtype=torch.float32, device=out.device)
    check(lib.gaot_scale_mix_fwd(_ptr_array(xs), len(xs), _ptr(logits), _ptr(out), _ptr(w), n, c, _stream()),
          "gaot_scale_mix_fwd")
    return out, w


def scale_mix_bwd(xs, w: Tensor, dout: Tensor):
    lib = _lib.load()
    n, c = xs[0].shape
    dxs = [torch.empty_like(x) for x in xs]
    dlog = torch.empty_like(w)
    check(lib.gaot_scale_mix_bwd(_ptr_array(xs), len(xs), _ptr(w), _ptr(dout), _ptr_array(dxs), _ptr(dlog), n, c,
                                 _stream()), "gaot_scale_mix_bwd")
    return dxs, dlog


def mlp2_forward(x: Tensor, w1: Tensor, b1: Tensor, w2: Tensor, b2: Optional[Tensor]) -> Tensor:
    lib = _lib.load()
    rows, hid, oc = x.shape[0], w1.shape[0], w2.shape[0]
    out = torch.empty(rows, oc, dtype=torch.float32, device=x.device)
    check(lib.gaot_mlp2_fwd(_ptr(x), rows, x.shape[1], hid, oc, _ptr(w1), _ptr(b1), _ptr(w2), _ptr(b2), _ptr(out), _stream()),
          "gaot_mlp2_fwd")
    return out


def mlp2_backward(x: Tensor, w1: Tensor, b1: Tensor, w2: Tensor, dout: Tensor):
    lib = _lib.load()
    rows, hid, oc = x.shape[0], w1.shape[0], w2.shape[0]
    dx = torch.empty_like(x)
    dw1, db1, dw2 = torch.empty_like(w1), torch.empty_like(b1), torch.empty_like(w2)
    ws = _ws(lib.gaot_mlp2_bwd_workspace_bytes(hid, oc), x.device)
    check(lib.gaot_mlp2_bwd(_ptr(x), rows, x.shape[1], hid, oc, _ptr(w1), _ptr(b1), _ptr(w2), _ptr(dout), _ptr(dx), _ptr(dw1),
                            _ptr(db1), _ptr(dw2), _ptr(ws), ws.numel(), _stream()), "gaot_mlp2_bwd")
    return dx, dw1, db1, dw2


def launch_count_reset() -> None:
    _lib.load().gaot_launch_count(1)


def launch_count() -> int:
    return int(_lib.load().gaot_launch_count(0))
```

include/gaot3d_hip.h:

```cpp
#ifndef GAOT3D_HIP_H
#define GAOT3D_HIP_H

#include <stddef.h>
#include <stdint.h>

#ifdef __cplusplus
extern "C" {
#endif

#define GAOT_OK 0
#define GAOT_ERR_ARG 1
#define GAOT_ERR_LAUNCH 2
#define GAOT_ERR_UNSUPPORTED 3

#define GAOT_ABI_VERSION 11
#define GAOT_MAX_MLP_LAYERS 5

typedef void* gaot_stream_t;

int gaot_abi_version(void);
const char* gaot_last_error(void);
int64_t gaot_launch_count(int reset);

size_t gaot_csr_workspace_bytes(int64_t num_edges, int64_t num_rows);
int gaot_csr_build(const void* edge_index, int index_is_i64, int64_t num_edges, int sort_row, int64_t num_rows,
                   int32_t* rowptr, int32_t* perm, int32_t* key_sorted, int32_t* other_sorted, void* workspace,
                   size_t workspace_bytes, gaot_stream_t stream);

typedef struct {
    int n_hidden;
    int hidden;
    int channels;
    const float* weight[GAOT_MAX_MLP_LAYERS];
    const float* bias[GAOT_MAX_MLP_LAYERS];
} gaot_mlp_t;

typedef struct {
    float* weight[GAOT_MAX_MLP_LAYERS];
    float* bias[GAOT_MAX_MLP_LAYERS];
} gaot_mlp_grad_t;

size_t gaot_gno_fwd_workspace_bytes(int64_t num_edges, int channels);
int gaot_gno_fwd(const gaot_mlp_t* mlp , const float* y_pos, const float* x_pos, const float* f_y,
                 const int32_t* src_sorted, const int32_t* dst_sorted, const int32_t* rowptr_dst, int64_t num_edges,
                 int64_t num_queries, float* out ,
                 int precision ,
                 void* workspace, size_t workspace_bytes, gaot_stream_t stream);

size_t gaot_gno_bwd_workspace_bytes(const gaot_mlp_t* mlp , int64_t num_edges, int64_t num_queries);
int gaot_gno_bwd(const gaot_mlp_t* mlp , const float* y_pos, const float* x_pos, const float* f_y,
                 const float* grad_out , const int32_t* rowptr_dst,
                 const int32_t* src_sorted , const int32_t* dst_sorted ,
                 const int32_t* rowptr_src, int64_t num_edges, int64_t num_sources, int64_t num_queries,
                 float* grad_f_y , const gaot_mlp_grad_t* grads ,
                 int precision, void* workspace, size_t workspace_bytes, gaot_stream_t stream);
int gaot_gno_bwd_coords(const gaot_mlp_t* mlp , const float* y_pos, const float* x_pos, const float* f_y,
                        const float* grad_out, const int32_t* rowptr_dst, const int32_t* src_sorted, const int32_t* dst_sorted,
                        const int32_t* rowptr_src, int64_t num_edges, int64_t num_sources, int64_t num_queries,
                        float* grad_f_y, const gaot_mlp_grad_t* grads , float* grad_edge_coords ,
                        int precision, void* workspace, size_t workspace_bytes, gaot_stream_t stream);

size_t gaot_geoembed_stats_workspace_bytes(void);
int gaot_geoembed_moments(const float* source_pos, const float* query_pos, const int32_t* rowptr_dst,
                          const int32_t* src_sorted, int64_t num_queries, double* moments, gaot_stream_t stream);
int gaot_geoembed_from_moments(const double* moments, int64_t num_queries, float* features, void* workspace,
                               size_t workspace_bytes, gaot_stream_t stream);
int gaot_geoembed_raw(const float* source_pos, const float* query_pos, const int32_t* rowptr_dst, const int32_t* src_sorted,
                      int64_t num_queries, float* features, double* colsums, void* workspace, size_t workspace_bytes,
                      gaot_stream_t stream);
int gaot_geoembed_finalize(float* features, int64_t num_queries, const double* colsums, int64_t num_queries_total,
                           void* workspace, size_t workspace_bytes, gaot_stream_t stream);
size_t gaot_geoembed_from_moments_bwd_workspace_bytes(int64_t num_queries);
int gaot_geoembed_from_moments_bwd(const double* moments, const float* grad_features, int64_t num_queries,
                                   double* grad_moments, void* workspace, size_t workspace_bytes, gaot_stream_t stream);
int gaot_geoembed_moments_bwd(const float* source_pos, const float* query_pos, const int32_t* rowptr_dst,
                              const int32_t* src_sorted, int64_t num_queries, const double* grad_moments,
                              float* grad_edge , float* grad_query , gaot_stream_t stream);

size_t gaot_gemm_workspace_bytes(int64_t M, int64_t N, int64_t K);
int gaot_gemm(const float* A, const float* B, float* C, int64_t M, int64_t N, int64_t K, int64_t lda, int64_t ldb,
              int64_t ldc, int a_trans, int b_trans, const float* bias, int act, const float* residual, int64_t ldr,
              float* preact, int precision, void* workspace, size_t workspace_bytes, gaot_stream_t stream);
int gaot_gemm_ex(const void* A, const void* B, void* C, int64_t M, int64_t N, int64_t K, int64_t lda, int64_t ldb,
                 int64_t ldc, int a_trans, int b_trans, int a_bf16, int b_bf16, int c_bf16, const float* bias, int act,
                 const float* residual, int64_t ldr, float* preact, int precision, void* workspace,
                 size_t workspace_bytes, gaot_stream_t stream);

int gaot_attn_fwd(const float* q, const float* k, const float* v, float* o, float* lse, int64_t ldq, int64_t ldk,
                  int64_t ldv, int64_t ldo, int B, int S, int H, int HKV, int head_dim, float scale, float dropout_p,
                  const unsigned long long* dropout_seed, int head0, int heads_total, int precision, gaot_stream_t stream);
int gaot_attn_bwd(const float* q, const float* k, const float* v, const float* o, const float* d_o, const float* lse,
                  float* delta, float* dq, float* dk, float* dv, int64_t ldq, int64_t ldk, int64_t ldv, int64_t ldo,
                  int64_t lddo, int64_t lddq, int64_t lddk, int64_t lddv, int B, int S, int H, int HKV, int head_dim,
                  float scale, float dropout_p, const unsigned long long* dropout_seed, int head0, int heads_total,
                  int precision, int phase_mask , gaot_stream_t stream);
int64_t gaot_attn_bwd_fused_f32_scratch_bytes(int B, int S, int H);
int gaot_attn_bwd_fused_f32(const float* q, const float* k, const float* v, const float* o, const float* d_o, const float* lse,
                            float* delta, float* dq, float* dk, float* dv, int64_t ldq, int64_t ldk, int64_t ldv, int64_t ldo,
                            int64_t lddo, int64_t lddq, int64_t lddk, int64_t lddv, int B, int S, int H, int HKV, int head_dim,
                            float scale, float dropout_p, const unsigned long long* dropout_seed, int head0, int heads_total,
                            int run_delta, void* scratch, size_t scratch_bytes, gaot_stream_t stream);
int gaot_attn_dropout_mask(const unsigned long long* dropout_seed, float dropout_p, int B, int H, int S,
                           unsigned char* keep, gaot_stream_t stream);
int gaot_dropout_seed_next(unsigned long long* state, unsigned long long stride, unsigned long long* out,
                           gaot_stream_t stream);
int gaot_dropout_seed_block(unsigned long long* state, unsigned long long stride, int n, unsigned long long* out, gaot_stream_t stream);

int gaot_rope_table(const float* freqs, int S, int half_dim, float* table, gaot_stream_t stream);
int gaot_qkv_image(const void* x_bf16, const void* w_bf16, void* image, int64_t rows, int64_t lda, int64_t ldw, int S, int H,
                   int HKV, const float* rope_table, float qscale, gaot_stream_t stream);
int gaot_qkv_image_packed(const void* x_bf16, const void* w_bf16, void* packed, int64_t rows, int64_t lda, int64_t ldw,
                          int64_t pos0, int H, int HKV, const float* rope_table, float qscale, int world, gaot_stream_t stream);
int gaot_pack_heads(void* rows_buf, void* blocks_buf, int64_t rows, int ld, int world, int nseg, const int* col0,
                    const int* width, int rows_dtype, int blocks_dtype, int to_blocks, gaot_stream_t stream);
size_t gaot_attn_bf16_image_bytes(int B, int S, int H, int HKV);
size_t gaot_attn_bwd_bf16_scratch_bytes(int B, int S, int H, int HKV);
int gaot_attn_bwd_bf16_fused_eligible(int B, int S, int H, int HKV);
int gaot_attn_fwd_bf16(const float* qkv, const float* rope_freqs, void* qkv_image, float* o, float* lse, int B, int S,
                       int H, int HKV, int head_dim, float scale, float dropout_p,
                       const unsigned long long* dropout_seed, int head0, int heads_total, gaot_stream_t stream);
int gaot_attn_bwd_bf16(const void* qkv_image, const float* o, const float* d_o, const float* lse, void* do_image,
                       float* delta, float* dqkv, const float* rope_freqs, int B, int S, int H, int HKV, int head_dim,
                       float scale, float dropout_p, const unsigned long long* dropout_seed, int head0, int heads_total,
                       int phase_mask, gaot_stream_t stream);

int gaot_rmsnorm_fwd(const float* x, const float* weight, float* y, float* rstd, void* y_bf16 , int64_t rows, int dim, float eps,
                     gaot_stream_t stream);
size_t gaot_rmsnorm_bwd_workspace_bytes(int64_t rows, int dim);
int gaot_rmsnorm_bwd(const float* x, const float* weight, const float* dy, const float* rstd, const float* dx_add,
                     float* dx, float* dweight, int64_t rows, int dim, void* workspace, size_t workspace_bytes,
                     gaot_stream_t stream);
int gaot_rmsnorm_bwd2(const float* x, const float* weight, const float* dy, const float* rstd, const float* dx_add,
                      const float* dx_add2, float* dx, float* dweight, int64_t rows, int dim, void* workspace, size_t workspace_bytes,
                      gaot_stream_t stream);
size_t gaot_colsum_workspace_bytes(int64_t M, int64_t N);
int gaot_colsum(const float* x, int64_t M, int64_t N, int64_t ld, float* out, void* workspace, size_t workspace_bytes,
                gaot_stream_t stream);
typedef struct {
    const float* part;
    float* out;
    int64_t n;
    int32_t parts;
    int32_t lanes;
} gaot_reduce_desc_t;
int gaot_gemm_ex_partials(const void* A, const void* B, void* C, int64_t M, int64_t N, int64_t K, int64_t lda, int64_t ldb,
                          int64_t ldc, int a_trans, int b_trans, int a_bf16, int b_bf16, int precision, void* workspace,
                          size_t workspace_bytes, int* splits_out, int* lanes_out, gaot_stream_t stream);
int64_t gaot_rmsnorm_bwd_parts(int64_t rows);
int64_t gaot_colsum_parts(int64_t M);
int gaot_reduce_multi(const gaot_reduce_desc_t* descs, int count, gaot_stream_t stream);
int gaot_rope(float* x, int64_t rows, int64_t ld, int col0, int nheads, int head_dim, int seq_len, const float* freqs,
              int inverse, gaot_stream_t stream);
int gaot_swiglu_fwd(const float* ag, float* u, int64_t rows, int F, gaot_stream_t stream);
int gaot_swiglu_bwd(const float* ag, const float* du, float* dag, int64_t rows, int F, gaot_stream_t stream);
int gaot_cast_bf16(const float* src, void* dst, int64_t n, gaot_stream_t stream);
typedef struct {
    const float* src;
    void* dst;
    int64_t numel;
} gaot_cast_tensor_t;
int gaot_cast_bf16_multi(const gaot_cast_tensor_t* tensors, int num_tensors, gaot_stream_t stream);
int gaot_cast_bf16_transpose_multi(const gaot_cast_tensor_t* tensors, const int* rows, const int* cols, int num_tensors,
                                   gaot_stream_t stream);
int gaot_swiglu_fwd_bf16(const void* ag, void* u, int64_t rows, int F, gaot_stream_t stream);
int gaot_ffn_w13_swiglu(const void* x_bf16, const void* w13_bf16, void* ag, void* u, int64_t rows, int64_t lda, int64_t ldw, int F,
                        gaot_stream_t stream);
int gaot_swiglu_bwd_bf16(const void* ag, const void* du, void* dag, int64_t rows, int F, gaot_stream_t stream);
int gaot_ffn_w2_bwd_swiglu(const void* dy_bf16, const void* w2t_bf16, const void* ag, void* dag, int64_t rows, int64_t lda,
                           int64_t ldw, int F, gaot_stream_t stream);
int64_t gaot_ffn_packed_bytes(int F, int with_backward);
int gaot_ffn_pack(const float* w13, const float* w2, int F, void* packed, int with_backward, gaot_stream_t stream);
typedef struct {
    const float* w13;
    const float* w2;
    void* packed;
} gaot_ffn_pack_t;
int gaot_ffn_pack_multi(const gaot_ffn_pack_t* items, int num, int F, int with_backward, gaot_stream_t stream);
int gaot_ffn_fwd(const void* x_bf16, const void* packed, const float* residual, int64_t ldr, float* y, void* ag, void* u, int64_t rows,
                 int F, gaot_stream_t stream);
int gaot_norm_ffn_fwd(const float* h, int64_t ldh, const float* norm_weight, float eps, const void* packed, float* y, void* yb,
                      float* rstd, int64_t rows, int F, gaot_stream_t stream);
typedef struct {
    const float* w13;
    const float* w2;
    const float* wo;
    void* packed;
} gaot_block_pack_t;
int64_t gaot_block_packed_bytes(int F);
int gaot_block_pack_multi(const gaot_block_pack_t* items, int num, int F, gaot_stream_t stream);
int gaot_block_tail_fwd(const float* attn_out, int64_t ldo, const float* x, int64_t ldx, const float* norm_weight, float eps,
                        const void* packed, float* h, float* y, void* yb, float* rstd, int64_t rows, int F, gaot_stream_t stream);
typedef struct {
    const float* w;
    void* packed;
} gaot_qkv_pack_t;
int64_t gaot_qkv_packed_bytes(int64_t N, int with_backward);
int gaot_qkv_pack_multi(const gaot_qkv_pack_t* items, int num, int64_t N, int with_backward, gaot_stream_t stream);
int gaot_norm_qkv_image(const float* x, int64_t ldx, const float* norm_weight, float eps, const void* packed, void* image, void* yb,
                        float* rstd, int64_t rows, int S, int H, int HKV, const float* rope_table, float qscale, gaot_stream_t stream);
int64_t gaot_skip_packed_bytes(void);
int gaot_skip_pack_multi(const gaot_qkv_pack_t* items, int num, gaot_stream_t stream);
int gaot_cat_norm_qkv_image(const float* xa, int64_t ldxa, const float* xb, int64_t ldxb, const void* skip_packed, const float* skip_bias,
                            float* x_out, const float* norm_weight, float eps, const void* packed, void* image, void* yb, float* rstd,
                            int64_t rows, int S, int H, int HKV, const float* rope_table, float qscale, gaot_stream_t stream);
int64_t gaot_norm_bwd_parts(int64_t rows);
int gaot_ffn_bwd_norm(const void* yb, const float* dy, const void* packed, const float* h, int64_t ldh, const float* norm_weight,
                      const float* rstd, void* dag, void* u, void* dyb, float* dh, float* dw_part, int64_t rows, int F, gaot_stream_t stream);
int gaot_qkv_bwd_norm(const float* dqkv, int64_t N, const void* packed, const float* x, int64_t ldx, const float* norm_weight,
                      const float* rstd, const float* dres, const float* dtap, float* dx, float* dw_part, int64_t rows, gaot_stream_t stream);
int gaot_qkv_bwd_norm_cat(const float* dqkv, int64_t N, const void* packed, const float* x, int64_t ldx, const float* norm_weight,
                          const float* rstd, const float* dres, const void* skip_packed, float* dx, float* dxa, float* dxb, int same,
                          float* dw_part, int64_t rows, gaot_stream_t stream);
int gaot_oproj_bwd_image(const float* dh, const float* attn_out, const void* packed, int F, void* do_image, float* delta, int64_t rows,
                         int S, gaot_stream_t stream);
int gaot_ffn_bwd_dag(const void* x_bf16, const float* dy, const void* packed, void* dag, void* u, void* dyb, int64_t rows, int F,
                     gaot_stream_t stream);
int gaot_ffn_bwd(const void* x_bf16, const float* dy, const void* packed, void* dag, void* u, void* dyb, float* dx, int add_dy,
                 int64_t rows, int F, gaot_stream_t stream);
int gaot_act_fwd(const float* z, float* h, int64_t n, int act, gaot_stream_t stream);
int gaot_act_bwd(const float* z, const float* dh, float* dz, int64_t n, int act, gaot_stream_t stream);
int gaot_axpy(const float* a, const float* b, float alpha, float* out, int64_t n, int64_t period, gaot_stream_t stream);
int gaot_stream_copy(const void* src, void* dst, int64_t bytes, gaot_stream_t stream);
int gaot_stream_copy_ex(const void* src, void* dst, int64_t bytes, int variant, gaot_stream_t stream);
int gaot_patchify(const float* src, float* dst, int B, int D, int H, int W, int P, int C, int to_tokens,
                  gaot_stream_t stream);
size_t gaot_mse_workspace_bytes(void);
int gaot_mse_fwd(const float* pred, const float* target, int64_t n, float* loss, void* workspace, size_t workspace_bytes,
                 gaot_stream_t stream);
int gaot_mse_bwd(const float* pred, const float* target, int64_t n, const float* grad_loss, float* dpred,
                 gaot_stream_t stream);

int gaot_scale_mix_fwd(const float* const* xs, int num_scales, const float* logits, float* out, float* weights,
                       int64_t n, int channels, gaot_stream_t stream);
int gaot_scale_mix_bwd(const float* const* xs, int num_scales, const float* weights, const float* dout,
                       float* const* dxs, float* dlogits, int64_t n, int channels, gaot_stream_t stream);

typedef struct {
    float* param;
    const float* grad;
    float* exp_avg;
    float* exp_avg_sq;
    int64_t numel;
} gaot_adamw_tensor_t;
int gaot_adamw_step(const gaot_adamw_tensor_t* tensors, int num_tensors, const float* lr, float* step, double beta1,
                    double beta2, double eps, double weight_decay, gaot_stream_t stream);

typedef struct {
    int32_t dims[3];
    float lo[3];
    float hi[3];
} gaot_grid_t;
int gaot_knn_grid(const float* pos, int64_t num_points, const gaot_grid_t* grid, const float* token_pos, int k,
                  int32_t* out_idx, gaot_stream_t stream);
int gaot_radius_grid_count(const float* pos, int64_t num_points, const gaot_grid_t* grid, const float* token_pos,
                           float radius, int cap, int32_t* counts, gaot_stream_t stream);
int gaot_radius_grid_fill(const float* pos, int64_t num_points, const gaot_grid_t* grid, const float* token_pos,
                          float radius, int cap, const int32_t* offsets, int32_t* out_point, int32_t* out_token,
                          gaot_stream_t stream);
int gaot_knn_brute(const float* pos, int64_t num_points, const float* token_pos, int64_t num_tokens, int k, int32_t* out_idx,
                   gaot_stream_t stream);
int gaot_radius_brute_count(const float* pos, int64_t num_points, const float* token_pos, int64_t num_tokens, float radius,
                            int cap, int32_t* counts, gaot_stream_t stream);
int gaot_radius_brute_fill(const float* pos, int64_t num_points, const float* token_pos, int64_t num_tokens, float radius,
                           int cap, const int32_t* offsets, int32_t* out_point, int32_t* out_token, gaot_stream_t stream);
size_t gaot_exclusive_scan_workspace_bytes(int64_t n);
int gaot_exclusive_scan_i32(const int32_t* in, int64_t n, int32_t* out, void* workspace, size_t workspace_bytes,
                            gaot_stream_t stream);
int gaot_segment_cap_flags(const int32_t* rowptr, const int32_t* key_sorted, int64_t n, int cap, int32_t* flags,
                           gaot_stream_t stream);
int gaot_unique_pair_flags(const int32_t* a, const int32_t* b, int64_t n, int32_t* flags, gaot_stream_t stream);
int gaot_random_keep_flags(const unsigned long long* seed, int64_t n, double keep_prob, int32_t* flags,
                           gaot_stream_t stream);
int gaot_dropout(const float* x, const uint64_t* seed, double p, int64_t n, float* out, gaot_stream_t stream);
int gaot_segment_random_cap_flags(const unsigned long long* seed, const int32_t* rowptr, const int32_t* key_sorted,
                                  int64_t n, int cap, int32_t* flags, gaot_stream_t stream);
int gaot_compact_pairs(const int32_t* a, const int32_t* b, const int32_t* flags, const int32_t* offsets, int64_t n,
                       int32_t* out_a, int32_t* out_b, gaot_stream_t stream);

int gaot_mlp2_fwd(const float* x, int64_t num_rows, int in_dim, int hidden, int out_dim, const float* w1, const float* b1,
                  const float* w2, const float* b2, float* out, gaot_stream_t stream);
size_t gaot_mlp2_bwd_workspace_bytes(int hidden, int out_dim);
int gaot_mlp2_bwd(const float* x, int64_t num_rows, int in_dim, int hidden, int out_dim, const float* w1, const float* b1,
                  const float* w2, const float* d_out, float* d_x, float* d_w1, float* d_b1, float* d_w2, void* workspace,
                  size_t workspace_bytes, gaot_stream_t stream);

int gaot_gather_rows(const float* table, int64_t ld, const int32_t* idx, int64_t num_edges, int channels, float* out,
                     int64_t ld_out, gaot_stream_t stream);
int gaot_segment_reduce(const float* vals, int64_t ld_vals, const int32_t* rowptr, const int32_t* map, int64_t num_rows,
                        int channels, int mode, float* out, int32_t* argmax, gaot_stream_t stream);
int gaot_segment_reduce_bwd(const float* d_out, const int32_t* key, const int32_t* rowptr, const int32_t* argmax,
                            int64_t num_rows, int64_t num_edges, int channels, int mode, float* d_vals,
                            gaot_stream_t stream);
int gaot_segment_softmax_fwd(const float* scores, const int32_t* rowptr, int64_t num_rows, float* w, gaot_stream_t stream);
int gaot_segment_softmax_bwd(const float* w, const float* dw, const int32_t* rowptr, int64_t num_rows, float* ds,
                             gaot_stream_t stream);
int gaot_edge_coords(const float* y_pos, const float* x_pos, const int32_t* src, const int32_t* dst, int64_t num_edges,
                     int mode, float* out, int64_t ld_out, gaot_stream_t stream);
int gaot_mul(const float* a, const float* b, int64_t rows, int channels, int b_is_row_scalar, float* out,
             gaot_stream_t stream);
int gaot_mul_rowsum(const float* a, const float* b, int64_t rows, int channels, float* out, gaot_stream_t stream);
int gaot_affine_cols(const float* x, const float* scale_minus_one, const float* bias, int64_t rows, int channels,
                     float* out, gaot_stream_t stream);

#ifdef __cplusplus
}
#endif
#endif
```

Before: 24.97 million points/s.

## Add fused concat-linear and token-head kernels for geoembed recovery paths

Adds a HIP kernel that computes a linear layer over several concatenated narrow inputs without materialising the concatenation, with a backward kernel that produces dx, per-block dW and db partials in one pass. Adds a fused token-head kernel that chains the geoembed MLP (9->64->32) with the recovery linear over [enc, geo], keeping intermediates in LDS. The encoder and decoder recovery paths route through these kernels, replacing several GEMM launches and intermediate tensors. The new kernels are fp32 FMA rather than the bf16 GEMM path, which may change numerics and could be slower on large row counts.

```diff
diff --git a/gaot_3d_amd/_lib.py b/gaot_3d_amd/_lib.py
--- a/gaot_3d_amd/_lib.py
+++ b/gaot_3d_amd/_lib.py
@@ -84,6 +84,12 @@
     "gaot_mlp2_fwd": (_i, [_p, _i64, _i, _i, _i, _p, _p, _p, _p, _p, _p]),
     "gaot_mlp2_bwd_workspace_bytes": (_sz, [_i, _i]),
     "gaot_mlp2_bwd": (_i, [_p, _i64, _i, _i, _i, _p, _p, _p, _p, _p, _p, _p, _p, _p, _sz, _p]),
+    "gaot_catlin_fwd": (_i, [_p, _p, _i, _i64, _i, _p, _p, _p, _p]),
+    "gaot_catlin_bwd_parts": (_i64, [_i64, _i, _i]),
+    "gaot_catlin_bwd": (_i, [_p, _p, _i, _i64, _i, _p, _p, _p, _p, _p, _p]),
+    "gaot_tokenhead_fwd": (_i, [_p, _p, _i64, _i, _i, _i, _p, _p, _p, _p, _p, _p, _p, _p, _p, _p]),
+    "gaot_tokenhead_bwd_parts": (_i64, [_i64]),
+    "gaot_tokenhead_bwd": (_i, [_p, _p, _i64, _i, _i, _i, _p, _p, _p, _p, _p, _p, _p, _p, _p]),
     "gaot_knn_grid": (_i, [_p, _i64, _p, _p, _i, _p, _p]),
     "gaot_radius_grid_count": (_i, [_p, _i64, _p, _p, _f, _i, _p, _p]),
     "gaot_radius_grid_fill": (_i, [_p, _i64, _p, _p, _f, _i, _p, _p, _p, _p]),
diff --git a/gaot_3d_amd/csrc/catlin.hip b/gaot_3d_amd/csrc/catlin.hip
--- /dev/null
+++ b/gaot_3d_amd/csrc/catlin.hip
@@ -0,0 +1,769 @@
+#include "common.h"
+
+namespace {
+
+constexpr int CL_MAXIN = GAOT_CATLIN_MAX_INPUTS;
+constexpr int CL_FWD_ROWS = 128;
+constexpr int bwd_rows(int n, int kp) { return n * kp <= 1024 ? 128 : 64; }
+constexpr int fwd_per_cu(int n) { return n == 32 ? 2 : 1; }
+constexpr int bwd_per_cu(int n, int kp) { return n == 32 && kp <= 16 ? 3 : 2; }
+
+struct CatIn {
+    const float* x[CL_MAXIN];
+    int w[CL_MAXIN], off[CL_MAXIN];
+    int lo[CL_MAXIN];
+    int n, K, vec;
+};
+struct CatOut { float* dx[CL_MAXIN]; };
+
+template <int TR, bool PAD8 = false>
+__device__ __forceinline__ void stage_inputs(const CatIn& in, int64_t row0, int64_t M, int KP, float* __restrict__ t, int ld) {
+    const int nrows = (int)std::min<int64_t>(TR, M - row0);
+#pragma unroll
+    for (int i = 0; i < CL_MAXIN; ++i) {
+        if (i >= in.n) break;
+        const int w = in.w[i], off = PAD8 ? in.lo[i] : in.off[i];
+        const float* __restrict__ src = in.x[i] + row0 * w;
+        if (in.vec) {
+            const int w4 = w >> 2;
+#pragma unroll 4
+            for (int e = threadIdx.x; e < TR * w4; e += 256) {
+                const int row = e / w4, c = e - row * w4;
+                float4 v = make_float4(0.f, 0.f, 0.f, 0.f);
+                if (row < nrows) v = *reinterpret_cast<const float4*>(src + (int64_t)e * 4);
+                *reinterpret_cast<float4*>(t + row * ld + off + 4 * c) = v;
+            }
+        } else {
+#pragma unroll 4
+            for (int e = threadIdx.x; e < TR * w; e += 256) {
+                const int row = e / w, c = e - row * w;
+                t[row * ld + off + c] = row < nrows ? src[e] : 0.f;
+            }
+        }
+    }
+    if (PAD8) {
+#pragma unroll
+        for (int i = 0; i < CL_MAXIN; ++i) {
+            if (i >= in.n) break;
+            const int w = in.w[i], pad = ((w + 7) & ~7) - w;
+            if (pad > 0)
+#pragma unroll 1
+                for (int e = threadIdx.x; e < TR * pad; e += 256) {
+                    const int row = e / pad, c = e - row * pad;
+                    t[row * ld + in.lo[i] + w + c] = 0.f;
+                }
+        }
+        return;
+    }
+    const int pad = KP - in.K;
+    if (pad > 0)
+#pragma unroll 1
+        for (int e = threadIdx.x; e < TR * pad; e += 256) {
+            const int row = e / pad, c = e - row * pad;
+            t[row * ld + in.K + c] = 0.f;
+        }
+}
+
+template <int J, int RG>
+__device__ __forceinline__ void rows_times_b(const float* __restrict__ a, int lda, const float* __restrict__ b, int ldb, int R,
+                                             int rr, int cg, float (&acc)[J][4]) {
+#pragma unroll 2
+    for (int r = 0; r < R; r += 4) {
+        float4 bv[4];
+#pragma unroll
+        for (int q = 0; q < 4; ++q) bv[q] = *reinterpret_cast<const float4*>(b + (r + q) * ldb + 4 * cg);
+#pragma unroll
+        for (int j = 0; j < J; ++j) {
+            const float4 av = *reinterpret_cast<const float4*>(a + (rr + RG * j) * lda + r);
+            const float as[4] = {av.x, av.y, av.z, av.w};
+#pragma unroll
+            for (int q = 0; q < 4; ++q) {
+                acc[j][0] = fmaf(as[q], bv[q].x, acc[j][0]);
+                acc[j][1] = fmaf(as[q], bv[q].y, acc[j][1]);
+                acc[j][2] = fmaf(as[q], bv[q].z, acc[j][2]);
+                acc[j][3] = fmaf(as[q], bv[q].w, acc[j][3]);
+            }
+        }
+    }
+}
+
+template <int J, int RG>
+__device__ __forceinline__ void rows_times_b_gemm_order(const float* __restrict__ a, int lda, const float* __restrict__ b, int ldb, int R,
+                                                        int rr, int cg, float (&acc)[J][4]) {
+#pragma unroll 1
+    for (int r = 0; r < R; r += 8) {
+        float4 bv[8];
+#pragma unroll
+        for (int q = 0; q < 8; ++q) bv[q] = *reinterpret_cast<const float4*>(b + (r + q) * ldb + 4 * cg);
+#pragma unroll
+        for (int j = 0; j < J; ++j) {
+            const float4 a0 = *reinterpret_cast<const float4*>(a + (rr + RG * j) * lda + r);
+            const float4 a1 = *reinterpret_cast<const float4*>(a + (rr + RG * j) * lda + r + 4);
+            const float as[8] = {a0.x, a1.x, a0.y, a1.y, a0.z, a1.z, a0.w, a1.w};
+#pragma unroll
+            for (int t = 0; t < 8; ++t) {
+                const int q = (t >> 1) + 4 * (t & 1);
+                acc[j][0] = fmaf(as[t], bv[q].x, acc[j][0]);
+                acc[j][1] = fmaf(as[t], bv[q].y, acc[j][1]);
+                acc[j][2] = fmaf(as[t], bv[q].z, acc[j][2]);
+                acc[j][3] = fmaf(as[t], bv[q].w, acc[j][3]);
+            }
+        }
+    }
+}
+
+template <int KB>
+__device__ __forceinline__ void outer_acc(const float* __restrict__ d, int ldd, const float* __restrict__ x, int ldx, int r0, int r1,
+                                          int rs, int ng, int kg, float (&acc)[4][KB], float (&dbv)[4]) {
+    float cs[4] = {0.f, 0.f, 0.f, 0.f};
+#pragma unroll 2
+    for (int r = r0; r < r1; r += rs) {
+        const float4 d4 = *reinterpret_cast<const float4*>(d + r * ldd + 4 * ng);
+        const float dv[4] = {d4.x, d4.y, d4.z, d4.w};
+        float xv[KB];
+#pragma unroll
+        for (int b = 0; b < KB; b += 4) {
+            const float4 x4 = *reinterpret_cast<const float4*>(x + r * ldx + KB * kg + b);
+            xv[b] = x4.x; xv[b + 1] = x4.y; xv[b + 2] = x4.z; xv[b + 3] = x4.w;
+        }
+#pragma unroll
+        for (int a = 0; a < 4; ++a) {
+            cs[a] += dv[a];
+#pragma unroll
+            for (int b = 0; b < KB; ++b) acc[a][b] = fmaf(dv[a], xv[b], acc[a][b]);
+        }
+    }
+#pragma unroll
+    for (int a = 0; a < 4; ++a) dbv[a] += cs[a];
+}
+
+template <int N>
+__global__ __launch_bounds__(256, fwd_per_cu(N)) void k_catlin_fwd(CatIn in, int64_t M, const float* __restrict__ W, const float* __restrict__ bias,
+                                                       float* __restrict__ y) {
+    constexpr int CG = N / 4, RG = 256 / CG, J = CL_FWD_ROWS / RG;
+    extern __shared__ __attribute__((aligned(16))) float fsm[];
+    const int n_in = in.n;
+    int KP8 = 0;
+#pragma unroll
+    for (int i = 0; i < CL_MAXIN; ++i)
+        if (i < n_in) KP8 = in.lo[i] + ((in.w[i] + 7) & ~7);
+    const int LD = KP8 + 4;
+    float* xs = fsm;
+    float* bs = fsm + CL_FWD_ROWS * LD;
+    for (int i = threadIdx.x; i < KP8 * N; i += 256) bs[i] = 0.f;
+    __syncthreads();
+#pragma unroll
+    for (int i = 0; i < CL_MAXIN; ++i) {
+        if (i >= n_in) break;
+        const int w = in.w[i];
+        for (int e = threadIdx.x; e < w * N; e += 256) {
+            const int k = e / N, n = e - k * N;
+            bs[(in.lo[i] + k) * N + n] = W[n * in.K + in.off[i] + k];
+        }
+    }
+    const int cg = threadIdx.x % CG, rr = threadIdx.x / CG;
+    float b4[4];
+#pragma unroll
+    for (int c = 0; c < 4; ++c) b4[c] = bias ? bias[4 * cg + c] : 0.f;
+    const int64_t tiles = (M + CL_FWD_ROWS - 1) / CL_FWD_ROWS;
+    for (int64_t tile = blockIdx.x; tile < tiles; tile += gridDim.x) {
+        const int64_t row0 = tile * CL_FWD_ROWS;
+        __syncthreads();
+        stage_inputs<CL_FWD_ROWS, true>(in, row0, M, KP8, xs, LD);
+        __syncthreads();
+        float yv[J][4];
+#pragma unroll
+        for (int i = 0; i < CL_MAXIN; ++i) {
+            if (i >= n_in) break;
+            float acc[J][4];
+#pragma unroll
+            for (int j = 0; j < J; ++j)
+#pragma unroll
+                for (int c = 0; c < 4; ++c) acc[j][c] = 0.f;
+            rows_times_b_gemm_order<J, RG>(xs + in.lo[i], LD, bs + in.lo[i] * N, N, (in.w[i] + 7) & ~7, rr, cg, acc);
+#pragma unroll
+            for (int j = 0; j < J; ++j)
+#pragma unroll
+                for (int c = 0; c < 4; ++c) yv[j][c] = i == 0 ? acc[j][c] + b4[c] : acc[j][c] + yv[j][c];
+        }
+#pragma unroll
+        for (int j = 0; j < J; ++j) {
+            const int64_t row = row0 + rr + RG * j;
+            if (row < M) *reinterpret_cast<float4*>(y + row * N + 4 * cg) = make_float4(yv[j][0], yv[j][1], yv[j][2], yv[j][3]);
+        }
+    }
+}
+
+template <int N, int KP>
+__global__ __launch_bounds__(256, bwd_per_cu(N, KP)) void k_catlin_bwd(CatIn in, int64_t M, const float* __restrict__ W, const float* __restrict__ dy,
+                                                    CatOut out, int want_dx, float* __restrict__ dw_part, float* __restrict__ db_part) {
+    constexpr int NG = N / 4, CL_BWD_ROWS = bwd_rows(N, KP);
+    constexpr int KB = (NG * KP / 8 <= 64) ? 8 : NG * KP / 64;
+    constexpr int KG = KP / KB, RL = 64 / (NG * KG);
+    constexpr int LDY = N + 4, LDX = KP + 4;
+    static_assert(NG * KG * RL == 64 && CL_BWD_ROWS % (4 * RL) == 0, "lane layout");
+    constexpr int TILE_FLOATS = CL_BWD_ROWS * (LDY + LDX) + N * KP, RED = N * KP + N;
+    static_assert(3 * RED <= TILE_FLOATS, "the waves' sums reuse the tiles' LDS");
+    __shared__ __attribute__((aligned(16))) float smem[TILE_FLOATS];
+    float* dys = smem;
+    float* xs = dys + CL_BWD_ROWS * LDY;
+    float* wd = xs + CL_BWD_ROWS * LDX;
+    const int K = in.K;
+    const int wave = threadIdx.x >> 6, lane = threadIdx.x & 63;
+    const int ng = lane % NG, kg = (lane / NG) % KG, rl = lane / (NG * KG);
+    if (want_dx)
+        for (int i = threadIdx.x; i < N * KP; i += 256) {
+            const int n = i / KP, k = i - n * KP;
+            wd[i] = k < K ? W[n * K + k] : 0.f;
+        }
+    float acc[4][KB], dbv[4];
+#pragma unroll
+    for (int a = 0; a < 4; ++a) {
+        dbv[a] = 0.f;
+#pragma unroll
+        for (int b = 0; b < KB; ++b) acc[a][b] = 0.f;
+    }
+    const int64_t tiles = (M + CL_BWD_ROWS - 1) / CL_BWD_ROWS;
+    for (int64_t tile = blockIdx.x; tile < tiles; tile += gridDim.x) {
+        const int64_t row0 = tile * CL_BWD_ROWS;
+        const int nrows = (int)std::min<int64_t>(CL_BWD_ROWS, M - row0);
+        __syncthreads();
+        stage_inputs<CL_BWD_ROWS>(in, row0, M, KP, xs, LDX);
+#pragma unroll 4
+        for (int e = threadIdx.x; e < CL_BWD_ROWS * NG; e += 256) {
+            const int row = e / NG, c = e - row * NG;
+            float4 v = make_float4(0.f, 0.f, 0.f, 0.f);
+            if (row < nrows) v = *reinterpret_cast<const float4*>(dy + (row0 + row) * N + 4 * c);
+            *reinterpret_cast<float4*>(dys + row * LDY + 4 * c) = v;
+        }
+        __syncthreads();
+        outer_acc<KB>(dys, LDY, xs, LDX, wave * RL + rl, CL_BWD_ROWS, 4 * RL, ng, kg, acc, dbv);
+        if (want_dx) {
+            constexpr int CG = KP / 4, RG = 256 / CG, J = CL_BWD_ROWS >= RG ? CL_BWD_ROWS / RG : 1;
+            const int cg = threadIdx.x % CG, rr = threadIdx.x / CG, k0 = 4 * cg;
+            int which = -1;
+#pragma unroll
+            for (int i = 0; i < CL_MAXIN; ++i)
+                if (i < in.n && k0 >= in.off[i] && k0 < in.off[i] + in.w[i] && out.dx[i]) which = i;
+            if (which >= 0 && rr < CL_BWD_ROWS) {
+                float a4[J][4];
+#pragma unroll
+                for (int j = 0; j < J; ++j)
+#pragma unroll
+                    for (int c = 0; c < 4; ++c) a4[j][c] = 0.f;
+                rows_times_b<J, RG>(dys, LDY, wd, KP, N, rr, cg, a4);
+                float* dst = nullptr;
+                int w = 0, off = 0;
+#pragma unroll
+                for (int i = 0; i < CL_MAXIN; ++i)
+                    if (i == which) { dst = out.dx[i]; w = in.w[i]; off = in.off[i]; }
+#pragma unroll
+                for (int j = 0; j < J; ++j) {
+                    const int r = rr + RG * j;
+                    if (r < nrows)
+                        *reinterpret_cast<float4*>(dst + (row0 + r) * w + (k0 - off)) = make_float4(a4[j][0], a4[j][1], a4[j][2], a4[j][3]);
+                }
+            }
+        }
+    }
+#pragma unroll
+    for (int o = NG * KG; o < 64; o <<= 1) {
+#pragma unroll
+        for (int a = 0; a < 4; ++a) {
+            dbv[a] += __shfl_xor(dbv[a], o, 64);
+#pragma unroll
+            for (int b = 0; b < KB; ++b) acc[a][b] += __shfl_xor(acc[a][b], o, 64);
+        }
+    }
+    __syncthreads();
+    if (rl == 0 && wave > 0) {
+        float* red = smem + (wave - 1) * RED;
+#pragma unroll
+        for (int a = 0; a < 4; ++a) {
+#pragma unroll
+            for (int b = 0; b < KB; ++b) red[(4 * ng + a) * KP + KB * kg + b] = acc[a][b];
+            if (kg == 0) red[N * KP + 4 * ng + a] = dbv[a];
+        }
+    }
+    __syncthreads();
+    if (rl == 0 && wave == 0) {
+        const int64_t p = blockIdx.x;
+#pragma unroll
+        for (int a = 0; a < 4; ++a) {
+            const int n = 4 * ng + a;
+            if (dw_part) {
+#pragma unroll
+                for (int b = 0; b < KB; ++b) {
+                    const int k = KB * kg + b, at = n * KP + k;
+                    if (k < K) dw_part[p * N * K + n * K + k] = ((acc[a][b] + smem[at]) + smem[RED + at]) + smem[2 * RED + at];
+                }
+            }
+            if (db_part && kg == 0)
+                db_part[p * N + n] = ((dbv[a] + smem[N * KP + n]) + smem[RED + N * KP + n]) + smem[2 * RED + N * KP + n];
+        }
+    }
+}
+
+constexpr int TH_F = 9, TH_H = 64, TH_C = 32;
+constexpr int TH_LDF = 20, TH_LDH = TH_H + 4, TH_LDC = TH_C + 4;
+constexpr int TH_GRID = 512;
+
+struct HeadArgs {
+    const float* feats; const float* enc; int64_t M;
+    const float *w0, *b0, *w2, *b2, *wr, *br;
+};
+
+template <int TR, int W>
+__device__ __forceinline__ void stage_rows4(const float* __restrict__ src, int64_t row0, int nrows, float* __restrict__ t, int ld, int col0) {
+#pragma unroll 2
+    for (int e = threadIdx.x; e < TR * (W / 4); e += 256) {
+        const int row = e / (W / 4), c = e % (W / 4);
+        float4 v = make_float4(0.f, 0.f, 0.f, 0.f);
+        if (row < nrows) v = *reinterpret_cast<const float4*>(src + (row0 + row) * W + 4 * c);
+        *reinterpret_cast<float4*>(t + row * ld + col0 + 4 * c) = v;
+    }
+}
+template <int TR>
+__device__ __forceinline__ void stage_feats(const float* __restrict__ feats, int64_t row0, int nrows, float* __restrict__ t) {
+#pragma unroll 2
+    for (int e = threadIdx.x; e < TR * 16; e += 256) {
+        const int row = e >> 4, c = e & 15;
+        t[row * TH_LDF + c] = (c < TH_F && row < nrows) ? feats[(row0 + row) * TH_F + c] : 0.f;
+    }
+}
+__device__ __forceinline__ void load_w0t(const float* __restrict__ w0, float* __restrict__ w0t) {
+    for (int i = threadIdx.x; i < 16 * TH_H; i += 256) {
+        const int k = i / TH_H, j = i % TH_H;
+        w0t[i] = k < TH_F ? w0[j * TH_F + k] : 0.f;
+    }
+}
+__device__ __forceinline__ void load_t64x32(const float* __restrict__ w, float* __restrict__ wt) {
+    for (int i = threadIdx.x; i < 64 * 32; i += 256) wt[i] = w[(i % 32) * 64 + i / 32];
+}
+__device__ __forceinline__ void load_32x64(const float* __restrict__ w, float* __restrict__ ws) {
+    for (int i = threadIdx.x; i < 32 * 64; i += 256) ws[i] = w[i];
+}
+
+__global__ __launch_bounds__(256, 2) void k_tokenhead_fwd(HeadArgs a, float* __restrict__ out, float* __restrict__ h_out,
+                                                          float* __restrict__ geo_out) {
+    constexpr int TR = 64;
+    __shared__ __attribute__((aligned(16))) float sm[TR * (TH_LDF + 2 * TH_LDH) + 16 * TH_H + 2 * 64 * 32];
+    float* F = sm;
+    float* CAT = F + TR * TH_LDF;
+    float* Hs = CAT + TR * TH_LDH;
+    float* w0t = Hs + TR * TH_LDH;
+    float* w2t = w0t + 16 * TH_H;
+    float* wrt = w2t + 64 * 32;
+    load_w0t(a.w0, w0t);
+    load_t64x32(a.w2, w2t);
+    load_t64x32(a.wr, wrt);
+    const int cg16 = threadIdx.x % 16, rr16 = threadIdx.x / 16;
+    const int cg8 = threadIdx.x % 8, rr32 = threadIdx.x / 8;
+    float b0v[4], b2v[4], brv[4];
+#pragma unroll
+    for (int c = 0; c < 4; ++c) {
+        b0v[c] = a.b0[4 * cg16 + c];
+        b2v[c] = a.b2[4 * cg8 + c];
+        brv[c] = a.br ? a.br[4 * cg8 + c] : 0.f;
+    }
+    const int64_t tiles = (a.M + TR - 1) / TR;
+    for (int64_t tile = blockIdx.x; tile < tiles; tile += gridDim.x) {
+        const int64_t row0 = tile * TR;
+        const int nrows = (int)std::min<int64_t>(TR, a.M - row0);
+        __syncthreads();
+        stage_feats<TR>(a.feats, row0, nrows, F);
+        stage_rows4<TR, TH_C>(a.enc, row0, nrows, CAT, TH_LDH, 0);
+        __syncthreads();
+        {
+            float acc[4][4];
+#pragma unroll
+            for (int j = 0; j < 4; ++j)
+#pragma unroll
+                for (int c = 0; c < 4; ++c) acc[j][c] = 0.f;
+            rows_times_b_gemm_order<4, 16>(F, TH_LDF, w0t, TH_H, 16, rr16, cg16, acc);
+#pragma unroll
+            for (int j = 0; j < 4; ++j) {
+                float v[4];
+#pragma unroll
+                for (int c = 0; c < 4; ++c) {
+                    v[c] = acc[j][c] + b0v[c];
+                    v[c] = v[c] > 0.f ? v[c] : 0.f;
+                }
+                const int r = rr16 + 16 * j;
+                const float4 h4 = make_float4(v[0], v[1], v[2], v[3]);
+                *reinterpret_cast<float4*>(Hs + r * TH_LDH + 4 * cg16) = h4;
+                if (h_out && r < nrows) *reinterpret_cast<float4*>(h_out + (row0 + r) * TH_H + 4 * cg16) = h4;
+            }
+        }
+        __syncthreads();
+        {
+            float acc[2][4];
+#pragma unroll
+            for (int j = 0; j < 2; ++j)
+#pragma unroll
+                for (int c = 0; c < 4; ++c) acc[j][c] = 0.f;
+            rows_times_b_gemm_order<2, 32>(Hs, TH_LDH, w2t, TH_C, TH_H, rr32, cg8, acc);
+#pragma unroll
+            for (int j = 0; j < 2; ++j) {
+                const int r = rr32 + 32 * j;
+                const float4 g4 = make_float4(acc[j][0] + b2v[0], acc[j][1] + b2v[1], acc[j][2] + b2v[2], acc[j][3] + b2v[3]);
+                *reinterpret_cast<float4*>(CAT + r * TH_LDH + TH_C + 4 * cg8) = g4;
+                if (geo_out && r < nrows) *reinterpret_cast<float4*>(geo_out + (row0 + r) * TH_C + 4 * cg8) = g4;
+            }
+        }
+        __syncthreads();
+        {
+            float y1[2][4], acc[2][4];
+#pragma unroll
+            for (int j = 0; j < 2; ++j)
+#pragma unroll
+                for (int c = 0; c < 4; ++c) y1[j][c] = 0.f;
+            rows_times_b_gemm_order<2, 32>(CAT, TH_LDH, wrt, TH_C, TH_C, rr32, cg8, y1);
+#pragma unroll
+            for (int j = 0; j < 2; ++j)
+#pragma unroll
+                for (int c = 0; c < 4; ++c) {
+                    y1[j][c] += brv[c];
+                    acc[j][c] = 0.f;
+                }
+            rows_times_b_gemm_order<2, 32>(CAT + TH_C, TH_LDH, wrt + TH_C * TH_C, TH_C, TH_C, rr32, cg8, acc);
+#pragma unroll
+            for (int j = 0; j < 2; ++j) {
+                const int r = rr32 + 32 * j;
+                if (r < nrows)
+                    *reinterpret_cast<float4*>(out + (row0 + r) * TH_C + 4 * cg8) =
+                        make_float4(acc[j][0] + y1[j][0], acc[j][1] + y1[j][1], acc[j][2] + y1[j][2], acc[j][3] + y1[j][3]);
+            }
+        }
+    }
+}
+
+constexpr int TH_NWR = 32 * 64, TH_NW0 = TH_H * TH_F;
+
+__global__ __launch_bounds__(256, 2) void k_tokenhead_bwd(HeadArgs a, const float* __restrict__ dout, float* __restrict__ d_enc,
+                                                          float* __restrict__ part) {
+    constexpr int TR = 32;
+    constexpr int RED_A = TH_NWR + 32, RED_B = TH_H * 16 + TH_H;
+    constexpr int SM_FLOATS = TR * (TH_LDF + 2 * TH_LDH + 2 * TH_LDC) + 16 * TH_H + 3 * 64 * 32;
+    static_assert(2 * RED_A + 3 * RED_B <= SM_FLOATS, "the waves' sums reuse the tiles' LDS");
+    __shared__ __attribute__((aligned(16))) float sm[SM_FLOATS];
+    float* F = sm;
+    float* CAT = F + TR * TH_LDF;
+    float* Hs = CAT + TR * TH_LDH;
+    float* D = Hs + TR * TH_LDH;
+    float* DG = D + TR * TH_LDC;
+    float* w0t = DG + TR * TH_LDC;
+    float* w2t = w0t + 16 * TH_H;
+    float* wrs = w2t + 64 * 32;
+    float* w2s = wrs + 32 * 64;
+    load_w0t(a.w0, w0t);
+    load_t64x32(a.w2, w2t);
+    load_32x64(a.wr, wrs);
+    load_32x64(a.w2, w2s);
+    const int wave = threadIdx.x >> 6, lane = threadIdx.x & 63;
+    const int cg16 = threadIdx.x % 16, rr16 = threadIdx.x / 16;
+    const int cg8 = threadIdx.x % 8, rr32 = threadIdx.x / 8;
+    const int ngA = lane % 8, kgA = lane / 8;
+    const int ngB = lane % 16, kgB = (lane / 16) % 2, rlB = lane / 32;
+    float b0v[4], b2v[4];
+#pragma unroll
+    for (int c = 0; c < 4; ++c) {
+        b0v[c] = a.b0[4 * cg16 + c];
+        b2v[c] = a.b2[4 * cg8 + c];
+    }
+    float accA[4][8], dbA[4], accB[4][8], dbB[4];
+#pragma unroll
+    for (int x = 0; x < 4; ++x) {
+        dbA[x] = dbB[x] = 0.f;
+#pragma unroll
+        for (int b = 0; b < 8; ++b) accA[x][b] = accB[x][b] = 0.f;
+    }
+    const int64_t tiles = (a.M + TR - 1) / TR;
+    for (int64_t tile = blockIdx.x; tile < tiles; tile += gridDim.x) {
+        const int64_t row0 = tile * TR;
+        const int nrows = (int)std::min<int64_t>(TR, a.M - row0);
+        __syncthreads();
+        stage_feats<TR>(a.feats, row0, nrows, F);
+        stage_rows4<TR, TH_C>(a.enc, row0, nrows, CAT, TH_LDH, 0);
+        stage_rows4<TR, TH_C>(dout, row0, nrows, D, TH_LDC, 0);
+        __syncthreads();
+        {
+            float acc[2][4];
+#pragma unroll
+            for (int j = 0; j < 2; ++j)
+#pragma unroll
+                for (int c = 0; c < 4; ++c) acc[j][c] = b0v[c];
+            rows_times_b<2, 16>(F, TH_LDF, w0t, TH_H, 12, rr16, cg16, acc);
+#pragma unroll
+            for (int j = 0; j < 2; ++j)
+                *reinterpret_cast<float4*>(Hs + (rr16 + 16 * j) * TH_LDH + 4 * cg16) =
+                    make_float4(fmaxf(acc[j][0], 0.f), fmaxf(acc[j][1], 0.f), fmaxf(acc[j][2], 0.f), fmaxf(acc[j][3], 0.f));
+        }
+        {
+            float acc[2][4];
+#pragma unroll
+            for (int j = 0; j < 2; ++j)
+#pragma unroll
+                for (int c = 0; c < 4; ++c) acc[j][c] = 0.f;
+            rows_times_b<2, 16>(D, TH_LDC, wrs, 2 * TH_C, TH_C, rr16, cg16, acc);
+#pragma unroll
+            for (int j = 0; j < 2; ++j) {
+                const int r = rr16 + 16 * j;
+                const float4 v = make_float4(acc[j][0], acc[j][1], acc[j][2], acc[j][3]);
+                if (cg16 >= 8) *reinterpret_cast<float4*>(DG + r * TH_LDC + 4 * (cg16 - 8)) = v;
+                else if (d_enc && r < nrows) *reinterpret_cast<float4*>(d_enc + (row0 + r) * TH_C + 4 * cg16) = v;
+            }
+        }
+        __syncthreads();
+        {
+            float acc[1][4];
+#pragma unroll
+            for (int c = 0; c < 4; ++c) acc[0][c] = b2v[c];
+            rows_times_b<1, 32>(Hs, TH_LDH, w2t, TH_C, TH_H, rr32, cg8, acc);
+            *reinterpret_cast<float4*>(CAT + rr32 * TH_LDH + TH_C + 4 * cg8) = make_float4(acc[0][0], acc[0][1], acc[0][2], acc[0][3]);
+        }
+        if (wave >= 2) outer_acc<8>(DG, TH_LDC, Hs, TH_LDH, wave & 1, TR, 2, ngA, kgA, accA, dbA);
+        __syncthreads();
+        if (wave < 2) outer_acc<8>(D, TH_LDC, CAT, TH_LDH, wave & 1, TR, 2, ngA, kgA, accA, dbA);
+        {
+            float acc[2][4];
+#pragma unroll
+            for (int j = 0; j < 2; ++j)
+#pragma unroll
+                for (int c = 0; c < 4; ++c) acc[j][c] = 0.f;
+            rows_times_b<2, 16>(DG, TH_LDC, w2s, TH_H, TH_C, rr16, cg16, acc);
+#pragma unroll
+            for (int j = 0; j < 2; ++j) {
+                float4* hp = reinterpret_cast<float4*>(Hs + (rr16 + 16 * j) * TH_LDH + 4 * cg16);
+                const float4 h = *hp;
+                *hp = make_float4(h.x > 0.f ? acc[j][0] : 0.f, h.y > 0.f ? acc[j][1] : 0.f, h.z > 0.f ? acc[j][2] : 0.f,
+                                  h.w > 0.f ? acc[j][3] : 0.f);
+            }
+        }
+        __syncthreads();
+        outer_acc<8>(Hs, TH_LDH, F, TH_LDF, 2 * wave + rlB, TR, 8, ngB, kgB, accB, dbB);
+    }
+#pragma unroll
+    for (int x = 0; x < 4; ++x) {
+        dbB[x] += __shfl_xor(dbB[x], 32, 64);
+#pragma unroll
+        for (int b = 0; b < 8; ++b) accB[x][b] += __shfl_xor(accB[x][b], 32, 64);
+    }
+    __syncthreads();
+    float* redA = sm + (wave >> 1) * RED_A;
+    float* redB = sm + 2 * RED_A;
+#pragma unroll
+    for (int x = 0; x < 4; ++x) {
+        if (wave & 1) {
+#pragma unroll
+            for (int b = 0; b < 8; ++b) redA[(4 * ngA + x) * 64 + 8 * kgA + b] = accA[x][b];
+            if (kgA == 0) redA[TH_NWR + 4 * ngA + x] = dbA[x];
+        }
+        if (wave > 0 && rlB == 0) {
+#pragma unroll
+            for (int b = 0; b < 8; ++b) redB[(wave - 1) * RED_B + (4 * ngB + x) * 16 + 8 * kgB + b] = accB[x][b];
+            if (kgB == 0) redB[(wave - 1) * RED_B + TH_H * 16 + 4 * ngB + x] = dbB[x];
+        }
+    }
+    __syncthreads();
+    const int64_t P = gridDim.x, p = blockIdx.x;
+    float* dw_ab = part + (wave >> 1) * P * RED_A;
+    float* dw0 = part + 2 * P * RED_A;
+    float* db0 = dw0 + P * TH_NW0;
+#pragma unroll
+    for (int x = 0; x < 4; ++x) {
+        if (!(wave & 1)) {
+            const int n = 4 * ngA + x;
+#pragma unroll
+            for (int b = 0; b < 8; ++b) {
+                const int at = n * 64 + 8 * kgA + b;
+                dw_ab[p * TH_NWR + at] = accA[x][b] + redA[at];
+            }
+            if (kgA == 0) dw_ab[P * TH_NWR + p * 32 + n] = dbA[x] + redA[TH_NWR + n];
+        }
+        if (wave == 0 && rlB == 0) {
+            const int n = 4 * ngB + x;
+#pragma unroll
+            for (int b = 0; b < 8; ++b) {
+                const int k = 8 * kgB + b, at = n * 16 + k;
+                if (k < TH_F) dw0[p * TH_NW0 + n * TH_F + k] = ((accB[x][b] + redB[at]) + redB[RED_B + at]) + redB[2 * RED_B + at];
+            }
+            if (kgB == 0) {
+                const int at = TH_H * 16 + n;
+                db0[p * TH_H + n] = ((dbB[x] + redB[at]) + redB[RED_B + at]) + redB[2 * RED_B + at];
+            }
+        }
+    }
+}
+
+int head_grid(int64_t rows, int tile) { return (int)std::max<int64_t>(1, std::min<int64_t>(ceil_div(rows, tile), TH_GRID)); }
+
+int check_head(int feat_dim, int hidden, int channels, const char* who) {
+    if (feat_dim != TH_F || hidden != TH_H || channels != TH_C) {
+        gaot_set_error("%s: supported shape is 9 features -> 64 hidden -> 32 channels (got %d -> %d -> %d)", who, feat_dim, hidden, channels);
+        return GAOT_ERR_UNSUPPORTED;
+    }
+    return GAOT_OK;
+}
+
+int fill_inputs(CatIn& in, const float* const* xs, const int* widths, int num_inputs, int64_t rows, const char* who) {
+    if (num_inputs < 1 || num_inputs > CL_MAXIN || !xs || !widths) {
+        gaot_set_error("%s: 1..%d inputs expected (got %d)", who, CL_MAXIN, num_inputs);
+        return GAOT_ERR_UNSUPPORTED;
+    }
+    in = CatIn{};
+    in.n = num_inputs;
+    in.vec = 1;
+    int k = 0, k8 = 0;
+    for (int i = 0; i < num_inputs; ++i) {
+        if (widths[i] < 1) {
+            gaot_set_error("%s: input %d has width %d", who, i, widths[i]);
+            return GAOT_ERR_ARG;
+        }
+        in.x[i] = xs[i];
+        in.w[i] = widths[i];
+        in.off[i] = k;
+        in.lo[i] = k8;
+        k8 += (widths[i] + 7) & ~7;
+        k += widths[i];
+        if (widths[i] % 4) in.vec = 0;
+        if (rows > 0 && !xs[i]) {
+            gaot_set_error("%s: null input %d", who, i);
+            return GAOT_ERR_ARG;
+        }
+    }
+    in.K = k;
+    if (k8 > 64) {
+        gaot_set_error("%s: total input width, each input rounded up to a multiple of 8, is %d > 64", who, k8);
+        return GAOT_ERR_UNSUPPORTED;
+    }
+    if (in.vec)
+        for (int i = 0; i < num_inputs; ++i)
+            if (((uintptr_t)xs[i] & 15) != 0) in.vec = 0;
+    return GAOT_OK;
+}
+
+int check_out(int out_dim, const char* who) {
+    if (out_dim != 32 && out_dim != 64) {
+        gaot_set_error("%s: output width must be 32 or 64 (got %d)", who, out_dim);
+        return GAOT_ERR_UNSUPPORTED;
+    }
+    return GAOT_OK;
+}
+
+int kp_of(int total_width) {
+    int kp = 8;
+    while (kp < total_width) kp <<= 1;
+    return kp;
+}
+int bwd_grid(int64_t rows, int total_width, int out_dim) {
+    const int tr = bwd_rows(out_dim, kp_of(total_width));
+    return (int)std::max<int64_t>(1, std::min<int64_t>(ceil_div(rows, tr), 256 * bwd_per_cu(out_dim, kp_of(total_width))));
+}
+size_t fwd_lds_bytes(int kp8, int n) { return sizeof(float) * ((size_t)CL_FWD_ROWS * (kp8 + 4) + (size_t)kp8 * n); }
+
+template <int N>
+void bwd_kp(int kp, int grid, hipStream_t st, const CatIn& in, int64_t M, const float* W, const float* dy, const CatOut& out,
+            int want_dx, float* dw_part, float* db_part) {
+    switch (kp) {
+        case 8: GAOT_KLAUNCH((k_catlin_bwd<N, 8>), dim3(grid), dim3(256), 0, st, in, M, W, dy, out, want_dx, dw_part, db_part); break;
+        case 16: GAOT_KLAUNCH((k_catlin_bwd<N, 16>), dim3(grid), dim3(256), 0, st, in, M, W, dy, out, want_dx, dw_part, db_part); break;
+        case 32: GAOT_KLAUNCH((k_catlin_bwd<N, 32>), dim3(grid), dim3(256), 0, st, in, M, W, dy, out, want_dx, dw_part, db_part); break;
+        default: GAOT_KLAUNCH((k_catlin_bwd<N, 64>), dim3(grid), dim3(256), 0, st, in, M, W, dy, out, want_dx, dw_part, db_part); break;
+    }
+}
+
+}
+
+extern "C" int gaot_catlin_fwd(const float* const* xs, const int* widths, int num_inputs, int64_t rows, int out_dim,
+                               const float* weight, const float* bias, float* y, gaot_stream_t stream) {
+    GAOT_ENTER();
+    GAOT_CHECK_ARG(rows >= 0, "negative size");
+    if (int rc = check_out(out_dim, __func__)) return rc;
+    CatIn in;
+    if (int rc = fill_inputs(in, xs, widths, num_inputs, rows, __func__)) return rc;
+    if (rows == 0) return GAOT_OK;
+    GAOT_CHECK_ARG(weight && y, "null pointer");
+    GAOT_CHECK_ARG(((uintptr_t)y & 15) == 0, "y must be 16-byte aligned");
+    hipStream_t st = (hipStream_t)stream;
+    const int grid = (int)std::min<int64_t>(ceil_div(rows, CL_FWD_ROWS), 256 * fwd_per_cu(out_dim));
+    const size_t lds = fwd_lds_bytes(in.lo[in.n - 1] + ((in.w[in.n - 1] + 7) & ~7), out_dim);
+    if (out_dim == 32) GAOT_KLAUNCH((k_catlin_fwd<32>), dim3(grid), dim3(256), lds, st, in, rows, weight, bias, y);
+    else GAOT_KLAUNCH((k_catlin_fwd<64>), dim3(grid), dim3(256), lds, st, in, rows, weight, bias, y);
+    GAOT_LAUNCH_CHECK();
+    return GAOT_OK;
+}
+
+extern "C" int64_t gaot_catlin_bwd_parts(int64_t rows, int total_width, int out_dim) { return bwd_grid(rows, total_width, out_dim); }
+
+extern "C" int gaot_catlin_bwd(const float* const* xs, const int* widths, int num_inputs, int64_t rows, int out_dim,
+                               const float* weight, const float* dy, float* const* dxs, float* dw_part, float* db_part,
+                               gaot_stream_t stream) {
+    GAOT_ENTER();
+    GAOT_CHECK_ARG(rows >= 0, "negative size");
+    if (int rc = check_out(out_dim, __func__)) return rc;
+    CatIn in;
+    if (int rc = fill_inputs(in, xs, widths, num_inputs, rows, __func__)) return rc;
+    CatOut out{};
+    int want_dx = 0;
+    for (int i = 0; i < num_inputs; ++i) {
+        out.dx[i] = dxs ? dxs[i] : nullptr;
+        if (out.dx[i]) {
+            want_dx = 1;
+            GAOT_CHECK_ARG(((uintptr_t)out.dx[i] & 15) == 0, "dx must be 16-byte aligned");
+        }
+    }
+    if (want_dx && rows > 0) {
+        for (int i = 0; i < num_inputs; ++i)
+            if (widths[i] % 4) {
+                gaot_set_error("%s: input gradients need every width to be a multiple of 4 (input %d: %d)", __func__, i, widths[i]);
+                return GAOT_ERR_UNSUPPORTED;
+            }
+        GAOT_CHECK_ARG(weight, "null pointer");
+    }
+    if (rows > 0) GAOT_CHECK_ARG(dy && ((uintptr_t)dy & 15) == 0, "dy must be non-null and 16-byte aligned");
+    if (rows == 0) want_dx = 0;
+    if (!want_dx && !dw_part && !db_part) return GAOT_OK;
+    hipStream_t st = (hipStream_t)stream;
+    const int kp = kp_of(in.K);
+    const int grid = bwd_grid(rows, in.K, out_dim);
+    if (out_dim == 32) bwd_kp<32>(kp, grid, st, in, rows, weight, dy, out, want_dx, dw_part, db_part);
+    else bwd_kp<64>(kp, grid, st, in, rows, weight, dy, out, want_dx, dw_part, db_part);
+    GAOT_LAUNCH_CHECK();
+    return GAOT_OK;
+}
+
+extern "C" int gaot_tokenhead_fwd(const float* feats, const float* enc, int64_t rows, int feat_dim, int hidden, int channels,
+                                  const float* w0, const float* b0, const float* w2, const float* b2, const float* wr, const float* br,
+                                  float* out, float* h_out, float* geo_out, gaot_stream_t stream) {
+    GAOT_ENTER();
+    GAOT_CHECK_ARG(rows >= 0, "negative size");
+    if (int rc = check_head(feat_dim, hidden, channels, __func__)) return rc;
+    if (rows == 0) return GAOT_OK;
+    GAOT_CHECK_ARG(feats && enc && w0 && b0 && w2 && b2 && wr && out, "null pointer");
+    GAOT_CHECK_ARG((((uintptr_t)enc | (uintptr_t)out | (uintptr_t)h_out | (uintptr_t)geo_out) & 15) == 0,
+                   "enc, out, h_out and geo_out must be 16-byte aligned");
+    HeadArgs a{feats, enc, rows, w0, b0, w2, b2, wr, br};
+    GAOT_KLAUNCH(k_tokenhead_fwd, dim3(head_grid(rows, 64)), dim3(256), 0, (hipStream_t)stream, a, out, h_out, geo_out);
+    GAOT_LAUNCH_CHECK();
+    return GAOT_OK;
+}
+
+extern "C" int64_t gaot_tokenhead_bwd_parts(int64_t rows) { return head_grid(rows, 32); }
+
+extern "C" int gaot_tokenhead_bwd(const float* feats, const float* enc, int64_t rows, int feat_dim, int hidden, int channels,
+                                  const float* w0, const float* b0, const float* w2, const float* b2, const float* wr,
+                                  const float* d_out, float* d_enc, float* part, gaot_stream_t stream) {
+    GAOT_ENTER();
+    GAOT_CHECK_ARG(rows >= 0, "negative size");
+    if (int rc = check_head(feat_dim, hidden, channels, __func__)) return rc;
+    GAOT_CHECK_ARG(w0 && b0 && w2 && b2 && wr && part, "null pointer");
+    if (rows > 0) {
+        GAOT_CHECK_ARG(feats && enc && d_out, "null pointer");
+        GAOT_CHECK_ARG((((uintptr_t)enc | (uintptr_t)d_out | (uintptr_t)d_enc) & 15) == 0, "enc, d_out and d_enc must be 16-byte aligned");
+    }
+    HeadArgs a{feats, enc, rows, w0, b0, w2, b2, wr, nullptr};
+    GAOT_KLAUNCH(k_tokenhead_bwd, dim3(head_grid(rows, 32)), dim3(256), 0, (hipStream_t)stream, a, d_out, d_enc, part);
+    GAOT_LAUNCH_CHECK();
+    return GAOT_OK;
+}
diff --git a/gaot_3d_amd/functional.py b/gaot_3d_amd/functional.py
--- a/gaot_3d_amd/functional.py
+++ b/gaot_3d_amd/functional.py
@@ -1089,6 +1089,31 @@
     return ba is bb and a.data_ptr() == b.data_ptr() and a.shape == b.shape and a.stride() == b.stride()
 
 
+_CATLIN = {"mode": int(os.environ.get("GAOT_CATLIN_FUSED", "1"))}
+
+
+def catlin_fused(mode) -> int:
+    prev, _CATLIN["mode"] = _CATLIN["mode"], int(mode)
+    return prev
+
+
+def _catlin_fused(ctx, weight: Tensor, w: Tensor, bias: Optional[Tensor], precision: Optional[int], xs2) -> bool:
+    if not _CATLIN["mode"] or ctx.dups:
+        return False
+    prec = (1 if ops.get_precision() == "bf16" else 0) if precision is None else precision
+    if prec != 0 or w.dtype != torch.float32 or not w.is_cuda or not weight.is_contiguous():
+        return False
+    if bias is not None and (bias.dtype != torch.float32 or not bias.is_contiguous()):
+        return False
+    if any(x.dim() != 2 or x.dtype != torch.float32 or not x.is_cuda or x.shape[0] != xs2[0].shape[0] for x in xs2):
+        return False
+    widths = [int(x.shape[1]) for x in xs2]
+    if not ops.catlin_supported(widths, int(w.shape[0])):
+        return False
+    ctx.fused_bwd = _CATLIN["mode"] >= 2 and not (any(ctx.needs_input_grad[3:]) and any(wd % 4 for wd in widths))
+    return True
+
+
 class CatLinearFn(Function):
 
     @staticmethod
@@ -1099,6 +1124,14 @@
         if sum(x.shape[1] for x in xs2) != k:
             raise GaotError(f"cat_linear: inputs have {sum(x.shape[1] for x in xs2)} features, weight expects {k}")
         m = xs2[0].shape[0]
+        ctx.dups = any(_same_view(xs[i], xs[j]) for i in range(len(xs)) for j in range(i))
+        ctx.params = (weight, bias)
+        if _catlin_fused(ctx, weight, w, bias, precision, xs2):
+            ctx.fused = True
+            ctx.save_for_backward(w, *xs2)
+            ctx.meta = (precision, weight.shape, bias is not None)
+            return ops.catlin_forward(xs2, w, bias)
+        ctx.fused = ctx.fused_bwd = False
         if all(x.shape[1] > 64 and x.shape[1] % 8 == 0 for x in xs2):
             w = _wb(w, precision)
         y = None
@@ -1110,7 +1143,6 @@
             col += ki
         ctx.save_for_backward(w, *xs2)
         ctx.meta = (precision, weight.shape, bias is not None)
-        ctx.dups = any(_same_view(xs[i], xs[j]) for i in range(len(xs)) for j in range(i))
         return y
 
     @staticmethod
@@ -1120,6 +1152,12 @@
         n, k = w.shape
         d = dy if dy.is_contiguous() else dy.contiguous()
         m = d.shape[0]
+        if ctx.fused and ctx.fused_bwd:
+            need_dw, need_db = ctx.needs_input_grad[0], has_bias and ctx.needs_input_grad[1]
+            weight, bias = ctx.params
+            defer = ops.defer_ok((weight if need_dw else None, bias if need_db else None)) if (need_dw or need_db) else False
+            dxs, dw, db = ops.catlin_backward(xs, w, d, ctx.needs_input_grad[3:], need_dw, need_db, defer=defer)
+            return (dw.view(wshape) if dw is not None else None, db, None, *dxs)
         dw = torch.empty(n, k, dtype=torch.float32, device=d.device) if ctx.needs_input_grad[0] else None
         dxs = []
         col = 0
@@ -1142,6 +1180,74 @@
         return (dw.view(wshape) if dw is not None else None, db, None, *dxs)
 
 
+class TokenHeadFn(Function):
+
+    @staticmethod
+    def forward(ctx, enc: Tensor, feats: Tensor, w0: Tensor, b0: Tensor, w2: Tensor, b2: Tensor, wr: Tensor, br: Optional[Tensor]):
+        e = enc if enc.is_contiguous() else enc.contiguous()
+        f = feats if feats.is_contiguous() else feats.contiguous()
+        ctx.params = (w0, b0, w2, b2, wr, br)
+        ctx.fused_bwd = _CATLIN["mode"] >= 2
+        out, h, geo = ops.tokenhead_forward(f, e, w0, b0, w2, b2, wr, br, save=not ctx.fused_bwd and any(ctx.needs_input_grad))
+        if ctx.fused_bwd:
+            ctx.save_for_backward(e, f, w0, b0, w2, b2, wr)
+        else:
+            ctx.save_for_backward(e, f, w0, w2, wr, h, geo)
+        return out
+
+    @staticmethod
+    def backward(ctx, dy: Tensor):
+        d = dy if dy.is_contiguous() else dy.contiguous()
+        need = ctx.needs_input_grad
+        if ctx.fused_bwd:
+            e, f, w0, b0, w2, b2, wr = ctx.saved_tensors
+            defer = ops.defer_ok(tuple(p for p, n in zip(ctx.params, need[2:]) if n and p is not None)) if any(need[2:]) else False
+            d_enc, dw0, db0, dw2, db2, dwr, dbr = ops.tokenhead_backward(f, e, w0, b0, w2, b2, wr, d, need[0], defer=defer)
+            grads = (dw0, db0, dw2, db2, dwr, dbr if ctx.params[5] is not None else None)
+            return (d_enc, None, *[g if n else None for g, n in zip(grads, need[2:])])
+        e, f, w0, w2, wr, h, geo = ctx.saved_tensors
+        p0, pb0, p2, pb2, _pr, pbr = ctx.params
+        m, c, hid, nf = d.shape[0], wr.shape[0], w0.shape[0], w0.shape[1]
+        d_enc = ops.gemm(d, wr, m, c, c, c, 2 * c, False, False, precision=0) if need[0] else None
+        d_geo = ops.gemm(d, wr[:, c:], m, c, c, c, 2 * c, False, False, precision=0)
+        dwr = dbr = None
+        if need[6]:
+            dwr = torch.empty(c, 2 * c, dtype=torch.float32, device=d.device)
+            ops.gemm(d, e, c, c, m, c, c, True, False, out=dwr, ldc=2 * c, precision=0)
+            ops.gemm(d, geo, c, c, m, c, c, True, False, out=dwr[:, c:], ldc=2 * c, precision=0)
+        if pbr is not None and need[7]:
+            dbr = ops.colsum(d, m, c, c)
+        dh = ops.gemm(d_geo, w2, m, hid, c, c, hid, False, False, precision=0)
+        dw2 = _dw_gemm(d_geo, h, c, hid, m, c, hid, 0, (p2,)) if need[4] else None
+        db2 = ops.colsum(d_geo, m, c, c, defer=ops.defer_ok((pb2,))) if need[5] else None
+        dz = ops.act_bwd(h, dh, ops.ACT["relu"])
+        dw0 = _dw_gemm(dz, f, hid, nf, m, hid, nf, 0, (p0,)) if need[2] else None
+        db0 = ops.colsum(dz, m, hid, hid, defer=ops.defer_ok((pb0,))) if need[3] else None
+        return d_enc, None, dw0, db0, dw2, db2, dwr, dbr
+
+
+def token_head_ok(enc: Tensor, feats: Tensor, params) -> bool:
+    w0, b0, w2, b2, wr, br = params
+    if not _CATLIN["mode"] or feats.requires_grad or b0 is None or b2 is None:
+        return False
+    if enc.dim() != 2 or feats.dim() != 2 or enc.dtype != torch.float32 or feats.dtype != torch.float32 or not enc.is_cuda \
+            or enc.shape[0] != feats.shape[0] or enc.shape[1] != 32:
+        return False
+    ps = [p for p in params if p is not None]
+    if any(p.dtype != torch.float32 or not p.is_contiguous() or not p.is_cuda for p in ps):
+        return False
+    if w0.dim() != 2 or w2.dim() != 2 or wr.dim() != 2 or tuple(w2.shape) != (32, 64) or tuple(wr.shape) != (32, 64) \
+            or w0.shape[0] != 64 or feats.shape[1] != w0.shape[1]:
+        return False
+    if tuple(b0.shape) != (64,) or tuple(b2.shape) != (32,) or (br is not None and tuple(br.shape) != (32,)):
+        return False
+    return ops.tokenhead_supported(int(feats.shape[1]), 64, 32)
+
+
+def token_head(enc: Tensor, feats: Tensor, w0, b0, w2, b2, wr, br) -> Tensor:
+    return TokenHeadFn.apply(enc, feats, w0, b0, w2, b2, wr, br)
+
+
 def cat_linear(xs, weight, bias=None, precision: Optional[int] = None) -> Tensor:
     return CatLinearFn.apply(weight, bias, precision, *xs)
 
diff --git a/gaot_3d_amd/model/layers/geoembed.py b/gaot_3d_amd/model/layers/geoembed.py
--- a/gaot_3d_amd/model/layers/geoembed.py
+++ b/gaot_3d_amd/model/layers/geoembed.py
@@ -53,14 +53,27 @@
                 graph=None, shard_group=None, sharded_queries_total: Optional[int] = None):
         if graph is None:
             graph = graph_for(edge_index.to(query_pos.device), source_pos.shape[0], query_pos.shape[0])
+        if self.method == "pointnet":
+            if shard_group is not None and coords_need_grad(source_pos, query_pos):
+                raise NotImplementedError("GeometricEmbedding: gradients with respect to the coordinates are not supported for "
+                                          "point-sharded samples (shard_group); detach the coordinates")
+            if shard_group is not None and sharded_queries_total is None:
+                return self._forward_pointnet_sharded(source_pos, query_pos, graph, shard_group)
+            return self._forward_pointnet(source_pos, query_pos, graph)
+        return self.mlp_of(self.features(source_pos, query_pos, edge_index, graph=graph, shard_group=shard_group,
+                                         sharded_queries_total=sharded_queries_total))
+
+    def mlp_of(self, feats):
+        h = GF.linear(feats, self.mlp[0].weight, self.mlp[0].bias, act="relu", precision=0)
+        return GF.linear(h, self.mlp[2].weight, self.mlp[2].bias, precision=0)
+
+    def features(self, source_pos, query_pos, edge_index, graph=None, shard_group=None, sharded_queries_total: Optional[int] = None):
+        if graph is None:
+            graph = graph_for(edge_index.to(query_pos.device), source_pos.shape[0], query_pos.shape[0])
         coord_grad = coords_need_grad(source_pos, query_pos)
         if shard_group is not None and coord_grad:
             raise NotImplementedError("GeometricEmbedding: gradients with respect to the coordinates are not supported for "
                                       "point-sharded samples (shard_group); detach the coordinates")
-        if self.method == "pointnet":
-            if shard_group is not None and sharded_queries_total is None:
-                return self._forward_pointnet_sharded(source_pos, query_pos, graph, shard_group)
-            return self._forward_pointnet(source_pos, query_pos, graph)
         if shard_group is not None and sharded_queries_total is not None:
             feats = ops.geoembed_stats_sharded_queries(source_pos, query_pos, graph, shard_group, sharded_queries_total)
         elif shard_group is not None:
@@ -79,8 +92,7 @@
             else:
                 feats = ops.geoembed_from_moments(ops.geoembed_moments(source_pos, query_pos, graph))
                 graph.__dict__["_geo_feats"] = (source_pos, source_pos._version, query_pos, query_pos._version, feats)
-        h = GF.linear(feats, self.mlp[0].weight, self.mlp[0].bias, act="relu", precision=0)
-        return GF.linear(h, self.mlp[2].weight, self.mlp[2].bias, precision=0)
+        return feats
 
     def _forward_pointnet_sharded(self, source_pos, query_pos, g, group):
         from ...sharding import GlobalSegmentMaxFn, GlobalSegmentMeanFn
diff --git a/gaot_3d_amd/model/layers/magno.py b/gaot_3d_amd/model/layers/magno.py
--- a/gaot_3d_amd/model/layers/magno.py
+++ b/gaot_3d_amd/model/layers/magno.py
@@ -163,6 +163,19 @@
     h = GF.linear(pos, sw[0].weight, sw[0].bias, act="relu", precision=0)
     logits = GF.linear(h, sw[2].weight, sw[2].bias, precision=0)
     return GF.ScaleMixFn.apply(logits, *outs)
+
+
+def _recover(mod, rows, source_pos, query_pos, edge_index, g, **kw):
+    ge, rec = mod.geoembed, mod.recovery.fcs[0]
+    if ge.method == "statistical" and mod.mlp_type == "linear":
+        feats = ge.features(source_pos, query_pos, edge_index, graph=g, **kw)
+        params = (ge.mlp[0].weight, ge.mlp[0].bias, ge.mlp[2].weight, ge.mlp[2].bias, rec.weight, rec.bias)
+        if GF.token_head_ok(rows, feats, params):
+            return GF.token_head(rows, feats, *params)
+        geo = ge.mlp_of(feats)
+    else:
+        geo = ge(source_pos, query_pos, edge_index, graph=g, **kw)
+    return GF.cat_linear([rows, geo], rec.weight, rec.bias, precision=0)
 
 
 class MAGNOEncoder(nn.Module):
@@ -250,12 +263,10 @@
                 from ...sharding import GlobalSegmentMeanFn
                 deg = (g.by_dst.rowptr[1:] - g.by_dst.rowptr[:-1]).to(enc.dtype)
                 enc = GlobalSegmentMeanFn.apply(enc, deg, shard_group)
-            geo = self.geoembed(phys_pos, latent_tokens_pos, edge_index, graph=g, shard_group=shard_group) \
-                if self.use_geoembed else None
-            if enc is not None and geo is not None:
-                enc = GF.cat_linear([enc, geo], self.recovery.fcs[0].weight, self.recovery.fcs[0].bias, precision=0)
-            elif enc is None and geo is not None:
-                enc = geo
+            if enc is not None and self.use_geoembed:
+                enc = _recover(self, enc, phys_pos, latent_tokens_pos, edge_index, g, shard_group=shard_group)
+            elif enc is None and self.use_geoembed:
+                enc = self.geoembed(phys_pos, latent_tokens_pos, edge_index, graph=g, shard_group=shard_group)
             elif enc is None:
                 raise ValueError("GNO and GeoEmbed are both disabled. No encoding will be performed.")
             outs.append(enc)
@@ -321,10 +332,9 @@
                 sg = getattr(self, "_shard_group", None)
                 if sg is not None:
                     total = getattr(batch, "shard", (0, 0, 0, 0, phys_pos_query.shape[0]))[4]
-                    geo = self.geoembed(latent_tokens_pos, phys_pos_query, edge_index, graph=g, shard_group=sg,
-                                        sharded_queries_total=total)
+                    dec = _recover(self, dec, latent_tokens_pos, phys_pos_query, edge_index, g, shard_group=sg,
+                                   sharded_queries_total=total)
                 else:
-                    geo = self.geoembed(latent_tokens_pos, phys_pos_query, edge_index, graph=g)
-                dec = GF.cat_linear([dec, geo], self.recovery.fcs[0].weight, self.recovery.fcs[0].bias, precision=0)
+                    dec = _recover(self, dec, latent_tokens_pos, phys_pos_query, edge_index, g)
             outs.append(dec)
         return self.projection.forward_rows(_mix_scales(self, outs, phys_pos_query))
diff --git a/gaot_3d_amd/ops.py b/gaot_3d_amd/ops.py
--- a/gaot_3d_amd/ops.py
+++ b/gaot_3d_amd/ops.py
@@ -1219,6 +1219,103 @@
     return dx, dw1, db1, dw2
 
 
+CATLIN_MAX_INPUTS = 4
+
+
+def catlin_supported(widths: Sequence[int], out_dim: int) -> bool:
+    return 1 <= len(widths) <= CATLIN_MAX_INPUTS and all(w >= 1 for w in widths) and sum((w + 7) // 8 * 8 for w in widths) <= 64 \
+        and out_dim in (32, 64)
+
+
+def _catlin_arrays(xs: Sequence[Tensor]):
+    n = len(xs)
+    return (C.c_void_p * n)(*[x.data_ptr() for x in xs]), (C.c_int * n)(*[int(x.shape[1]) for x in xs])
+
+
+def catlin_forward(xs: Sequence[Tensor], weight: Tensor, bias: Optional[Tensor]) -> Tensor:
+    lib = _lib.load()
+    xs = [_req(x, torch.float32, "x") for x in xs]
+    w = _req(weight, torch.float32, "weight")
+    b = _req(bias, torch.float32, "bias") if bias is not None else None
+    rows, n = xs[0].shape[0], w.shape[0]
+    y = torch.empty(rows, n, dtype=torch.float32, device=xs[0].device)
+    ptrs, widths = _catlin_arrays(xs)
+    check(lib.gaot_catlin_fwd(ptrs, widths, len(xs), rows, n, _ptr(w), _ptr(b), _ptr(y), _stream()), "gaot_catlin_fwd")
+    return y
+
+
+def catlin_backward(xs: Sequence[Tensor], weight: Tensor, dy: Tensor, need_dx: Sequence[bool], need_dw: bool, need_db: bool,
+                    defer: bool = False):
+    lib = _lib.load()
+    xs = [_req(x, torch.float32, "x") for x in xs]
+    w = _req(weight, torch.float32, "weight")
+    d = _req(dy, torch.float32, "dy")
+    rows, (n, k) = xs[0].shape[0], w.shape
+    dev = d.device
+    dxs = [torch.empty_like(x) if need else None for x, need in zip(xs, need_dx)]
+    parts = int(lib.gaot_catlin_bwd_parts(rows, k, n))
+    dwp = torch.empty(parts, n * k, dtype=torch.float32, device=dev) if need_dw else None
+    dbp = torch.empty(parts, n, dtype=torch.float32, device=dev) if need_db else None
+    ptrs, widths = _catlin_arrays(xs)
+    dptrs = (C.c_void_p * len(xs))(*[t.data_ptr() if t is not None else None for t in dxs])
+    check(lib.gaot_catlin_bwd(ptrs, widths, len(xs), rows, n, _ptr(w), _ptr(d), dptrs, _ptr(dwp), _ptr(dbp), _stream()),
+          "gaot_catlin_bwd")
+    dw = torch.empty(n, k, dtype=torch.float32, device=dev) if need_dw else None
+    db = torch.empty(n, dtype=torch.float32, device=dev) if need_db else None
+    _reduce_tables([(p, o) for p, o in ((dwp, dw), (dbp, db)) if o is not None], parts, defer)
+    return dxs, dw, db
+
+
+def _reduce_tables(tables, parts: int, defer: bool) -> None:
+    if defer:
+        for p, o in tables:
+            _defer(p, o, o.numel(), parts, 32)
+    elif tables:
+        arr = (_ReduceDesc * len(tables))()
+        for i, (p, o) in enumerate(tables):
+            arr[i].part, arr[i].out, arr[i].n, arr[i].parts, arr[i].lanes = p.data_ptr(), o.data_ptr(), o.numel(), parts, 32
+        check(_lib.load().gaot_reduce_multi(arr, len(tables), _stream()), "gaot_reduce_multi")
+
+
+def tokenhead_supported(feat_dim: int, hidden: int, channels: int) -> bool:
+    return (feat_dim, hidden, channels) == (9, 64, 32)
+
+
+def tokenhead_forward(feats: Tensor, enc: Tensor, w0: Tensor, b0: Tensor, w2: Tensor, b2: Tensor, wr: Tensor,
+                      br: Optional[Tensor], save: bool = False):
+    lib = _lib.load()
+    f, e = _req(feats, torch.float32, "feats"), _req(enc, torch.float32, "enc")
+    rows, dev = e.shape[0], e.device
+    out = torch.empty(rows, wr.shape[0], dtype=torch.float32, device=dev)
+    h = torch.empty(rows, w0.shape[0], dtype=torch.float32, device=dev) if save else None
+    geo = torch.empty(rows, w2.shape[0], dtype=torch.float32, device=dev) if save else None
+    check(lib.gaot_tokenhead_fwd(_ptr(f), _ptr(e), rows, f.shape[1], w0.shape[0], wr.shape[0], _ptr(w0), _ptr(b0), _ptr(w2), _ptr(b2),
+                                 _ptr(wr), _ptr(br), _ptr(out), _ptr(h), _ptr(geo), _stream()), "gaot_tokenhead_fwd")
+    return out, h, geo
+
+
+def tokenhead_backward(feats: Tensor, enc: Tensor, w0: Tensor, b0: Tensor, w2: Tensor, b2: Tensor, wr: Tensor, dout: Tensor,
+                       need_denc: bool, defer: bool = False):
+    lib = _lib.load()
+    f, e, d = _req(feats, torch.float32, "feats"), _req(enc, torch.float32, "enc"), _req(dout, torch.float32, "dout")
+    rows, dev = e.shape[0], e.device
+    hid, nf, c = w0.shape[0], w0.shape[1], wr.shape[0]
+    d_enc = torch.empty_like(e) if need_denc else None
+    parts = int(lib.gaot_tokenhead_bwd_parts(rows))
+    sizes = [c * 2 * c, c, c * hid, c, hid * nf, hid]
+    ws = torch.empty(parts * sum(sizes), dtype=torch.float32, device=dev)
+    check(lib.gaot_tokenhead_bwd(_ptr(f), _ptr(e), rows, nf, hid, c, _ptr(w0), _ptr(b0), _ptr(w2), _ptr(b2), _ptr(wr), _ptr(d),
+                                 _ptr(d_enc), _ptr(ws), _stream()), "gaot_tokenhead_bwd")
+    outs = [torch.empty(s, dtype=torch.float32, device=dev) for s in ((c, 2 * c), (c,), (c, hid), (c,), (hid, nf), (hid,))]
+    tables, at = [], 0
+    for n, o in zip(sizes, outs):
+        tables.append((ws[at:at + parts * n], o))
+        at += parts * n
+    _reduce_tables(tables, parts, defer)
+    dwr, dbr, dw2, db2, dw0, db0 = outs
+    return d_enc, dw0, db0, dw2, db2, dwr, dbr
+
+
 def launch_count_reset() -> None:
     _lib.load().gaot_launch_count(1)
 
diff --git a/include/gaot3d_hip.h b/include/gaot3d_hip.h
--- a/include/gaot3d_hip.h
+++ b/include/gaot3d_hip.h
@@ -284,6 +284,21 @@
                   const float* w2, const float* d_out, float* d_x, float* d_w1, float* d_b1, float* d_w2, void* workspace,
                   size_t workspace_bytes, gaot_stream_t stream);
 
+#define GAOT_CATLIN_MAX_INPUTS 4
+int gaot_catlin_fwd(const float* const* xs, const int* widths, int num_inputs, int64_t rows, int out_dim, const float* weight,
+                    const float* bias, float* y, gaot_stream_t stream);
+int64_t gaot_catlin_bwd_parts(int64_t rows, int total_width, int out_dim);
+int gaot_catlin_bwd(const float* const* xs, const int* widths, int num_inputs, int64_t rows, int out_dim, const float* weight,
+                    const float* dy, float* const* dxs, float* dw_part, float* db_part, gaot_stream_t stream);
+
+int gaot_tokenhead_fwd(const float* feats, const float* enc, int64_t rows, int feat_dim, int hidden, int channels, const float* w0,
+                       const float* b0, const float* w2, const float* b2, const float* wr, const float* br, float* out,
+                       float* h_out, float* geo_out, gaot_stream_t stream);
+int64_t gaot_tokenhead_bwd_parts(int64_t rows);
+int gaot_tokenhead_bwd(const float* feats, const float* enc, int64_t rows, int feat_dim, int hidden, int channels, const float* w0,
+                       const float* b0, const float* w2, const float* b2, const float* wr, const float* d_out, float* d_enc,
+                       float* part, gaot_stream_t stream);
+
 int gaot_gather_rows(const float* table, int64_t ld, const int32_t* idx, int64_t num_edges, int channels, float* out,
                      int64_t ld_out, gaot_stream_t stream);
 int gaot_segment_reduce(const float* vals, int64_t ld_vals, const int32_t* rowptr, const int32_t* map, int64_t num_rows,
```

Result: no change. 24.87 million points/s (-0.4%).
